# opencv/opencv_contrib

Hardware: AMD Instinct MI355X
Metric: frame-pairs/sec dense TV-L1 flow @1080p (higher is better)
Workload: dtype f32; 1 GPU; DualTVL1 dense flow, 1920x1080 CV_32FC1, 64 pairs/GPU/step (BASELINE configs[1]; 64 pairs/GPU = the per-GPU share of ~; warps=5, nscales=5, semantics=CPU_REF, math=fast, lanes=2

## Files before the change

### opencv_contrib_amd/csrc/mi_common.cpp

```cpp
#include "mi_common.h"
#include <vector>
#include <cstdlib>
#include <cstring>
#include <cstdio>
#include <mutex>

namespace mi {
static Tuning g_tuning;
static std::once_flag g_tuning_once;
static int env_int(const char *name, int dflt)
{
    const char *e = getenv(name);
    return e && *e ? atoi(e) : dflt;
}
#ifdef MIFLOW_EXPERIMENTS
#define EXP_INT(name, dflt) env_int(name, dflt)
#define EXP_ENV(name) getenv(name)
#else
#define EXP_INT(name, dflt) (dflt)
#define EXP_ENV(name) ((const char *)nullptr)
#endif
#ifndef MIFLOW_EXPERIMENTS
extern "C" char **environ;
static void warn_unread_switches()
{
    static const char *const known[] = {"MIFLOW_BF_W", "MIFLOW_CACHE_GB", "MIFLOW_CACHE_TOTAL_GB", "MIFLOW_FB_FUSE", "MIFLOW_FB_GROUP_MB", "MIFLOW_FB_NARROW",
                                        "MIFLOW_FB_PAIR", "MIFLOW_LANES", "MIFLOW_MULTI_RCCL", "MIFLOW_SURF_NMS0", "MIFLOW_SURF_POLY", "MIFLOW_SURF_STAGE_S",
                                        "MIFLOW_TB_HIST", "MIFLOW_TB_VERBOSE", "MIFLOW_TILE_MAXPX"};
    static const char *const foreign[] = {"MIFLOW_LIB", "MIFLOW_BENCH_", "MIFLOW_SWEEP_", "MIFLOW_BUILD_", "MIFLOW_EXTRA_", "MIFLOW_SLP_"};
    if (!environ) return;
    for (char **e = environ; *e; ++e) {
        if (strncmp(*e, "MIFLOW_", 7) != 0) continue;
        const char *eq = strchr(*e, '=');
        const size_t n = eq ? (size_t)(eq - *e) : strlen(*e);
        bool ok = false;
        for (const char *k : known) ok = ok || (strlen(k) == n && strncmp(k, *e, n) == 0);
        for (const char *k : foreign) ok = ok || strncmp(k, *e, strlen(k)) == 0;
        if (!ok) fprintf(stderr, "miflow: %.*s is not read by this library (tuning experiments exist in the -DMIFLOW_EXPERIMENTS build only); ignored\n", (int)n, *e);
    }
}
#endif
const Tuning &tuning()
{
    std::call_once(g_tuning_once, [] {
        Tuning &t = g_tuning;
#ifndef MIFLOW_EXPERIMENTS
        warn_unread_switches();
#endif
        t.x_skip = EXP_INT("MIFLOW_X_SKIP", 0);
        t.warp_tile = EXP_INT("MIFLOW_WARP_TILE", 32);
        if (t.warp_tile != 64 && t.warp_tile != 32 && t.warp_tile != 16) t.warp_tile = 32;
        t.warp_lds = EXP_INT("MIFLOW_WARP_LDS", 0);
        t.warp_fast = EXP_INT("MIFLOW_WARP_FAST", -1);
        t.warp_np = EXP_INT("MIFLOW_WARP_NP", 2);
        if (t.warp_np != 1 && t.warp_np != 4) t.warp_np = 2;
        t.tb_swz = EXP_INT("MIFLOW_TB_SWZ", 1);
        t.tb_p16 = EXP_INT("MIFLOW_TB_P16", 0);
        t.tb_nograd = EXP_INT("MIFLOW_TB_NOGRAD", 1);
        t.tb_skip_p = EXP_INT("MIFLOW_TB_SKIP_P", 1);
        t.tb_hist = env_int("MIFLOW_TB_HIST", 1);
        t.fb_poll = EXP_INT("MIFLOW_FB_POLL", 1);
        t.fb_ahead = EXP_INT("MIFLOW_FB_AHEAD", 1);
        t.tb_fw = EXP_INT("MIFLOW_TB_FW", 0);
        t.tb_jw = EXP_INT("MIFLOW_TB_JW", 2);
        if (t.tb_jw < 0 || t.tb_jw > 4) t.tb_jw = 2;
        t.tb_jw_spec = EXP_INT("MIFLOW_TB_JW_SPEC", 1);
        t.tb_ppl = t.tb_wps = t.tb_pf = -1;
        if (const char *v = EXP_ENV("MIFLOW_TB_VARIANT")) (void)sscanf(v, "%d,%d,%d", &t.tb_ppl, &t.tb_wps, &t.tb_pf);
        t.tb_force = EXP_ENV("MIFLOW_TB_FORCE") != nullptr;
        t.tb_plan_wps = EXP_INT("MIFLOW_TB_WPS", 0);
        t.tb_rows = EXP_INT("MIFLOW_TB_ROWS", 0);
        t.tb_verbose = getenv("MIFLOW_TB_VERBOSE") != nullptr;
        {
            const char *e = getenv("MIFLOW_TILE_MAXPX");
            t.tile_maxpx = e && *e ? atoll(e) : 2300000;
        }
        t.tile_variant = EXP_INT("MIFLOW_TILE_VARIANT", -1);
        t.tile_small_wgs = EXP_INT("MIFLOW_TILE_SMALL_WGS", 1024);
        t.tile_swz = EXP_INT("MIFLOW_TILE_SWZ", 1);
        t.warp_swz = EXP_INT("MIFLOW_WARP_SWZ", 1);
        t.tile_fb_block = EXP_INT("MIFLOW_TILE_FB_BLOCK", 10);
        t.tile_fb_model = EXP_INT("MIFLOW_TILE_FB_MODEL", 7);
        t.tile_spec = EXP_INT("MIFLOW_TILE_SPEC", 1);
        t.lanes = env_int("MIFLOW_LANES", 0);
        t.spec = EXP_INT("MIFLOW_SPEC", 1);
        t.exact_tb = EXP_INT("MIFLOW_EXACT_TB", 1);
        t.fb_tiled = EXP_INT("MIFLOW_FB_TILED", 1);
        t.sbm_wt = EXP_INT("MIFLOW_SBM_WT", 1);
        t.sbm_swz = EXP_INT("MIFLOW_SBM_SWZ", 1);
        t.sbm_texfuse = EXP_INT("MIFLOW_SBM_TEXFUSE", 1);
        t.fb_rows = EXP_INT("MIFLOW_FB_ROWS", 4) == 8 ? 8 : 4;
        t.fb_group_mb = env_int("MIFLOW_FB_GROUP_MB", 240);
        t.fb_fuse = env_int("MIFLOW_FB_FUSE", -1);
        t.fb_pair = env_int("MIFLOW_FB_PAIR", -1);
        t.fb_narrow = env_int("MIFLOW_FB_NARROW", -1);
        t.fb_swz = EXP_INT("MIFLOW_FB_SWZ", 1);
        t.fb_group_streams = EXP_INT("MIFLOW_FB_GROUP_STREAMS", 2);
        t.fb_poly_tiled = EXP_INT("MIFLOW_FB_POLY_TILED", 1);
        t.fb_direct = EXP_INT("MIFLOW_FB_DIRECT", 1);
        t.fb_blur_tiled = EXP_INT("MIFLOW_FB_BLUR_TILED", 1);
    });
    return g_tuning;
}

namespace {
struct BigBlock { void *p; size_t cap; int dev; hipEvent_t ready; };
std::mutex g_big_mu;
std::vector<BigBlock> g_big;
const size_t kBigMaxBlocks = 4;
size_t big_max_bytes()
{
    static const size_t v = [] {
        const char *e = getenv("MIFLOW_CACHE_GB");
        const long long gb = e && *e ? atoll(e) : 24;
        return (size_t)(gb < 0 ? 0 : gb) << 30;
    }();
    return v;
}
size_t big_max_bytes_total()
{
    static const size_t v = [] {
        const char *e = getenv("MIFLOW_CACHE_TOTAL_GB");
        if (e && *e) { const long long gb = atoll(e); return (size_t)(gb < 0 ? 0 : gb) << 30; }
        return 4 * big_max_bytes();
    }();
    return v;
}
}

int big_alloc(void **p, size_t bytes, size_t *capacity)
{
    int dev = 0;
    MI_HIP_TRY(hipGetDevice(&dev));
    {
        hipEvent_t ready = nullptr;
        bool hit = false;
        {
            std::lock_guard<std::mutex> lk(g_big_mu);
            int best = -1;
            for (size_t i = 0; i < g_big.size(); ++i)
                if (g_big[i].dev == dev && g_big[i].cap >= bytes && g_big[i].cap <= bytes + bytes / 2 + (64u << 20) &&
                    (best < 0 || g_big[i].cap < g_big[best].cap))
                    best = (int)i;
            if (best >= 0) {
                *p = g_big[best].p; *capacity = g_big[best].cap; ready = g_big[best].ready;
                g_big.erase(g_big.begin() + best);
                hit = true;
            }
        }
        if (hit) {
            if (ready) {
                const hipError_t we = hipEventSynchronize(ready);
                (void)hipEventDestroy(ready);
                if (we != hipSuccess) {
                    (void)hipGetLastError();
                    if (hipDeviceSynchronize() != hipSuccess) { (void)hipGetLastError(); (void)hipFree(*p); *p = nullptr; hit = false; }
                }
            }
            if (hit) return MI_OK;
        }
    }
    hipError_t e = hipMalloc(p, bytes);
    if (e != hipSuccess) {
        big_trim();
        e = hipMalloc(p, bytes);
    }
    if (e != hipSuccess) { set_error("hipMalloc of %zu bytes failed: %s", bytes, hipGetErrorString(e)); return MI_ERR_OOM; }
    *capacity = bytes;
    return MI_OK;
}

void big_free(void *p, size_t capacity, hipEvent_t ready, bool busy)
{
    if (!p) { if (ready) (void)hipEventDestroy(ready); return; }
    int dev = 0;
    void *drop = nullptr;
    if (hipGetDevice(&dev) == hipSuccess) {
        hipPointerAttribute_t at;
        const int cur = dev;
        if (hipPointerGetAttributes(&at, p) == hipSuccess) dev = at.device;
        if (dev != cur) (void)hipSetDevice(dev);
        bool idle = true;
        if (!ready && busy) idle = hipDeviceSynchronize() == hipSuccess;
        if (dev != cur) (void)hipSetDevice(cur);
        std::lock_guard<std::mutex> lk(g_big_mu);
        size_t total = capacity, all = capacity, blocks = 0;
        for (const BigBlock &b : g_big) {
            all += b.cap;
            if (b.dev == dev) { total += b.cap; ++blocks; }
        }
        if (idle && blocks < kBigMaxBlocks && total <= big_max_bytes() && all <= big_max_bytes_total()) {
            g_big.push_back({p, capacity, dev, ready});
            return;
        }
        if (ready) { (void)hipEventSynchronize(ready); (void)hipEventDestroy(ready); }
        drop = p;
    } else {
        if (ready) (void)hipEventDestroy(ready);
        drop = p;
    }
    const hipError_t fe = hipFree(drop);
    if (fe != hipSuccess) set_error("hipFree of a %zu-byte arena failed: %s", capacity, hipGetErrorString(fe));
}

void big_trim()
{
    std::vector<BigBlock> all;
    {
        std::lock_guard<std::mutex> lk(g_big_mu);
        all.swap(g_big);
    }
    int cur = 0;
    const bool have = hipGetDevice(&cur) == hipSuccess;
    for (const BigBlock &b : all) {
        if (b.ready) { (void)hipEventSynchronize(b.ready); (void)hipEventDestroy(b.ready); }
        (void)hipFree(b.p);
    }
    if (have) (void)hipSetDevice(cur);
}

int device_simds()
{
    static std::mutex mu;
    static int cache[64];
    int dev = 0;
    if (hipGetDevice(&dev) != hipSuccess || dev < 0 || dev >= 64) return 1024;
    std::lock_guard<std::mutex> lk(mu);
    if (!cache[dev]) {
        int cus = 0;
        if (hipDeviceGetAttribute(&cus, hipDeviceAttributeMultiprocessorCount, dev) != hipSuccess || cus <= 0) cus = 256;
        cache[dev] = 4 * cus;
    }
    return cache[dev];
}

static thread_local char g_err[512] = "";
void set_error(const char *fmt, ...)
{
    va_list ap;
    va_start(ap, fmt);
    vsnprintf(g_err, sizeof(g_err), fmt, ap);
    va_end(ap);
}
}

extern "C" {

const char *mi_last_error(void) { return mi::g_err; }
#ifdef MIFLOW_EXPERIMENTS
const char *mi_version(void) { return "miflow 0.1 (gfx950) +experiments"; }
#else
const char *mi_version(void) { return "miflow 0.1 (gfx950)"; }
#endif

int mi_device_count(void)
{
    int n = 0;
    if (hipGetDeviceCount(&n) != hipSuccess) return 0;
    return n;
}
int mi_set_device(int device) { MI_HIP_TRY(hipSetDevice(device)); return MI_OK; }
int mi_release_cached_memory(void) { mi::big_trim(); return MI_OK; }
int mi_get_device(int *device) { MI_REQUIRE(device, MI_ERR_BAD_ARG, "null device"); MI_HIP_TRY(hipGetDevice(device)); return MI_OK; }

int mi_malloc(void **dptr, size_t bytes)
{
    MI_REQUIRE(dptr, MI_ERR_BAD_ARG, "null dptr");
    MI_HIP_TRY(hipMalloc(dptr, bytes ? bytes : 1));
    return MI_OK;
}
int mi_malloc_pitch(void **dptr, size_t *step, size_t width_bytes, int rows)
{
    MI_REQUIRE(dptr && step && rows >= 0, MI_ERR_BAD_ARG, "bad mi_malloc_pitch arguments");
    const size_t st = rows > 1 ? (width_bytes + 255) / 256 * 256 : width_bytes;
    MI_HIP_TRY(hipMalloc(dptr, st * (size_t)(rows ? rows : 1) + 16));
    *step = st;
    return MI_OK;
}
int mi_free(void *dptr) { MI_HIP_TRY(hipFree(dptr)); return MI_OK; }
int mi_memcpy_h2d(void *dst, size_t dstep, const void *src, size_t sstep, size_t width_bytes, int rows, void *stream)
{
    MI_HIP_TRY(hipMemcpy2DAsync(dst, dstep, src, sstep, width_bytes, (size_t)rows, hipMemcpyHostToDevice, (hipStream_t)stream));
    return MI_OK;
}
int mi_memcpy_d2h(void *dst, size_t dstep, const void *src, size_t sstep, size_t width_bytes, int rows, void *stream)
{
    MI_HIP_TRY(hipMemcpy2DAsync(dst, dstep, src, sstep, width_bytes, (size_t)rows, hipMemcpyDeviceToHost, (hipStream_t)stream));
    return MI_OK;
}
int mi_memset(void *dst, size_t dstep, int value, size_t width_bytes, int rows, void *stream)
{
    MI_HIP_TRY(hipMemset2DAsync(dst, dstep, value, width_bytes, (size_t)rows, (hipStream_t)stream));
    return MI_OK;
}
int mi_stream_create(void **stream)
{
    MI_REQUIRE(stream, MI_ERR_BAD_ARG, "null stream");
    hipStream_t s;
    MI_HIP_TRY(hipStreamCreateWithFlags(&s, hipStreamNonBlocking));
    *stream = (void *)s;
    return MI_OK;
}
int mi_stream_destroy(void *stream) { MI_HIP_TRY(hipStreamDestroy((hipStream_t)stream)); return MI_OK; }
int mi_stream_synchronize(void *stream) { MI_HIP_TRY(hipStreamSynchronize((hipStream_t)stream)); return MI_OK; }

}
```

### opencv_contrib_amd/csrc/mi_common.h

```cpp
#pragma once
#include <vector>
#include <hip/hip_runtime.h>
#include <cstdarg>
#include <cstdio>
#include <cstring>
#include "miflow/c_api.h"

namespace mi {

void set_error(const char *fmt, ...);

#define MI_HIP_TRY(expr)                                                                  \
    do {                                                                                  \
        hipError_t _e = (expr);                                                           \
        if (_e != hipSuccess) {                                                           \
            mi::set_error("%s failed: %s (%s:%d)", #expr, hipGetErrorString(_e), __FILE__, __LINE__); \
            return _e == hipErrorOutOfMemory ? MI_ERR_OOM : MI_ERR_HIP;                   \
        }                                                                                 \
    } while (0)

#define MI_REQUIRE(cond, code, ...)        \
    do {                                   \
        if (!(cond)) {                     \
            mi::set_error(__VA_ARGS__);    \
            return (code);                 \
        }                                  \
    } while (0)

struct Tuning {
    int x_skip;
    int warp_tile;
    int warp_lds;
    int warp_fast;
    int warp_np;
    int tb_swz;
    int tb_p16;
    int tb_nograd;
    int tb_hist;
    int fb_poll;
    int fb_ahead;
    int tb_skip_p;
    int tb_fw;
    int tb_jw;
    int tb_jw_spec;
    int tb_ppl, tb_wps, tb_pf;
    int tb_force;
    int tb_plan_wps;
    int tb_rows;
    int tb_verbose;
    long long tile_maxpx;
    int tile_spec;
    int tile_variant;
    int tile_fb_block;
    int tile_fb_model;
    int tile_swz, warp_swz;
    int tile_small_wgs;
    int lanes;
    int exact_tb;
    int spec;
    int sbm_texfuse;
    int sbm_swz;
    int sbm_wt;
    int fb_rows, fb_swz;
    int fb_group_mb;
    int fb_fuse;
    int fb_pair;
    int fb_narrow;
    int fb_group_streams;
    int fb_poly_tiled;
    int fb_direct;
    int fb_blur_tiled;
    int fb_tiled;
};
const Tuning &tuning();
#ifdef MIFLOW_EXPERIMENTS
#define MI_EXP_ENV(name) getenv(name)
#else
#define MI_EXP_ENV(name) ((const char *)nullptr)
#endif

struct DevTmp {
    std::vector<void *> bufs;
    DevTmp() = default;
    DevTmp(const DevTmp &) = delete;
    DevTmp &operator=(const DevTmp &) = delete;
    ~DevTmp() { for (void *p : bufs) (void)hipFree(p); }
    template <class T>
    hipError_t alloc(T **out, size_t n)
    {
        void *p = nullptr;
        const hipError_t e = hipMalloc(&p, sizeof(T) * n);
        if (e == hipSuccess) bufs.push_back(p);
        *out = (T *)p;
        return e;
    }
};
int big_alloc(void **p, size_t bytes, size_t *capacity);
void big_free(void *p, size_t capacity, hipEvent_t ready = nullptr, bool busy = true);
void big_trim();
int device_simds();

static inline int div_up(int a, int b) { return (a + b - 1) / b; }
static inline int align_up(int a, int b) { return div_up(a, b) * b; }

struct PlaneF {
    float *p;
    int ld;
};

}
```

### opencv_contrib_amd/csrc/tvl1_api.cpp

```cpp
#include "tvl1_dev.h"
#include "mi_selftest.h"
#include <cfloat>
#include <algorithm>
#include <cmath>
#include <vector>
#include <chrono>
#include <sched.h>
#include <time.h>

using namespace mi;
using namespace mi::tvl1;

namespace {

constexpr double kFeedbackWaitLimitUs = 30e6;

struct LevelBuf {
    Geo g;
    float *I0 = nullptr, *I1 = nullptr;
    float *u[2][3] = {{nullptr, nullptr, nullptr}, {nullptr, nullptr, nullptr}};
};

struct SlotInfo { int scale, warp; };

template <class T, bool Host = false, unsigned HostFlags = 0>
struct GrowBuf {
    T *p = nullptr;
    size_t n = 0;
    GrowBuf() = default;
    GrowBuf(const GrowBuf &) = delete;
    ~GrowBuf() { release(); }
    int ensure(size_t want)
    {
        if (n >= want) return MI_OK;
        release();
        void *q = nullptr;
        if (Host) MI_HIP_TRY(hipHostMalloc(&q, sizeof(T) * want, HostFlags));
        else MI_HIP_TRY(hipMalloc(&q, sizeof(T) * want));
        p = (T *)q; n = want;
        return MI_OK;
    }
    void release()
    {
        if (p) (void)(Host ? hipHostFree(p) : hipFree(p));
        p = nullptr; n = 0;
    }
};

}

struct Lane {
    int capW = 0, capH = 0, capB = 0, capScales = 0;
    double capStep = 0;
    bool capGamma = false, capMedian = false;
    float *arena = nullptr;
    size_t arena_bytes = 0;
    std::vector<LevelBuf> L;
    float *scr[6] = {};
    float *pbuf[2][6] = {};
    GrowBuf<PtrTab> tab;
    std::vector<PtrTab> tab_host;
    GrowBuf<int2> S;
    GrowBuf<unsigned long long> E;
    GrowBuf<double> Pd;
    GrowBuf<int4> X;
    long long Q = 0;
    int ctlB = 0;
    GrowBuf<int> H;
    unsigned long long H_sig = 0;
    int H_par = 0;
    std::vector<SlotInfo> slots;
    GrowBuf<int2, true, hipHostMallocDefault> fb_host;
    hipEvent_t fb_ev = nullptr;
    GrowBuf<int, true, hipHostMallocCoherent | hipHostMallocMapped> fb_flag;
    int fb_seq = 0;
    std::vector<int> fb_hist;
    unsigned long long fb_hist_sig = 0;
    std::vector<hipEvent_t> ev_pool;
    struct Region { int e0, e1; long long launches; double bytes; int kind; int level; };
    std::vector<Region> regions;
    hipStream_t stream = nullptr;
    hipEvent_t done = nullptr;
    hipEvent_t idle_ev = nullptr;
    bool idle_valid = false;
    bool used = false;
};

struct mi_tvl1 {
    mi_tvl1_params P;
    int device = 0;
    float *cubic_tab = nullptr;
    static const int kMaxLanes = 4;
    Lane lane[kMaxLanes];
    hipEvent_t fork = nullptr;
    int last_nscales = 0, last_batch = 0, last_lanes = 1;
    int last_first[kMaxLanes + 1] = {};
    bool last_check = false;
    bool profiling = false;
};

void mi_tvl1_default_params(mi_tvl1_params *p)
{
    if (!p) return;
    p->tau = 0.25; p->lambda = 0.15; p->theta = 0.3; p->epsilon = 0.01; p->scale_step = 0.8; p->gamma = 0.0;
    p->nscales = 5; p->warps = 5; p->iterations = 300; p->use_initial_flow = 0;
    p->inner_iterations = 1; p->median_filtering = 1;
    p->semantics = MI_SEM_CPU_REF; p->exact_math = 0; p->time_block = 0; p->lanes = 0; p->stop_slack = 0; p->host_feedback = 0;
}

static const long long kMaxSlots = 4000000;

static int validate_params(const mi_tvl1_params *p)
{
    MI_REQUIRE(p, MI_ERR_BAD_ARG, "null params");
    MI_REQUIRE(p->nscales > 0 && p->nscales <= 32, MI_ERR_BAD_ARG, "nscales must be in [1,32] (CV_Assert nscales_ > 0)");
    MI_REQUIRE(p->warps >= 0 && p->warps <= 64, MI_ERR_BAD_ARG, "warps must be in [0,64]");
    MI_REQUIRE(p->iterations >= 0 && p->inner_iterations >= 0, MI_ERR_BAD_ARG, "negative iteration count");
    MI_REQUIRE((long long)p->iterations * p->inner_iterations <= kMaxSlots, MI_ERR_BAD_ARG,
               "iterations x inner_iterations must not exceed %lld", kMaxSlots);
    MI_REQUIRE(p->scale_step > 0 && p->scale_step < 1, MI_ERR_BAD_ARG, "scale_step must be in (0,1)");
    MI_REQUIRE(p->theta != 0, MI_ERR_BAD_ARG, "theta must be non-zero");
    MI_REQUIRE(p->semantics == MI_SEM_CPU_REF || p->semantics == MI_SEM_CUDA_COMPAT, MI_ERR_BAD_ARG, "bad semantics");
    MI_REQUIRE(p->median_filtering <= 1 || p->median_filtering == 3 || p->median_filtering == 5, MI_ERR_BAD_ARG,
               "medianFiltering must be 1 (off), 3 or 5 (cv::medianBlur on CV_32F)");
    MI_REQUIRE(p->lanes >= 0 && p->lanes <= 4, MI_ERR_BAD_ARG, "lanes must be 0 (automatic) or 1..4");
    MI_REQUIRE(p->stop_slack >= 0 && p->stop_slack <= 8, MI_ERR_BAD_ARG, "stop_slack must be in 0..8");
    MI_REQUIRE(p->host_feedback >= -1 && p->host_feedback <= 1, MI_ERR_BAD_ARG, "host_feedback must be -1, 0 or 1");
    return MI_OK;
}

int mi_tvl1_create(const mi_tvl1_params *p, mi_tvl1 **out)
{
    MI_REQUIRE(out, MI_ERR_BAD_ARG, "null out");
    *out = nullptr;
    mi_tvl1_params d;
    if (!p) { mi_tvl1_default_params(&d); p = &d; }
    int rc = validate_params(p);
    if (rc) return rc;
    int n = 0;
    if (hipGetDeviceCount(&n) != hipSuccess || n == 0) {
        set_error("no HIP device available: the miflow product path has no CPU fallback");
        return MI_ERR_NO_DEVICE;
    }
    mi_tvl1 *h = new mi_tvl1();
    h->P = *p;
    float tab[128];
    host_cubic_table(tab);
    auto upload = [&]() -> int {
        MI_HIP_TRY(hipGetDevice(&h->device));
        MI_HIP_TRY(hipMalloc((void **)&h->cubic_tab, sizeof(tab)));
        MI_HIP_TRY(hipMemcpy(h->cubic_tab, tab, sizeof(tab), hipMemcpyHostToDevice));
        return MI_OK;
    };
    if (const int rc = upload()) { mi_tvl1_destroy(h); return rc; }
    *out = h;
    return MI_OK;
}

int mi_tvl1_set_params(mi_tvl1 *h, const mi_tvl1_params *p)
{
    MI_REQUIRE(h, MI_ERR_BAD_ARG, "null handle");
    int rc = validate_params(p);
    if (rc) return rc;
    h->P = *p;
    return MI_OK;
}

int mi_tvl1_get_params(const mi_tvl1 *h, mi_tvl1_params *p)
{
    MI_REQUIRE(h && p, MI_ERR_BAD_ARG, "null argument");
    *p = h->P;
    return MI_OK;
}

static void free_arena(Lane &ln)
{
    if (ln.arena) {
        big_free(ln.arena, ln.arena_bytes, ln.idle_valid ? ln.idle_ev : nullptr, ln.used);
        if (ln.idle_valid) ln.idle_ev = nullptr;
    }
    ln.idle_valid = false;
    ln.used = false;
    ln.arena = nullptr;
    ln.L.clear();
}

int mi_tvl1_query_plan(int width, int height, int pairs_per_lane, int iterations_per_launch, int *kernel, int *rows_per_band)
{
    MI_REQUIRE(kernel && rows_per_band, MI_ERR_BAD_ARG, "null output");
    MI_REQUIRE(width > 0 && height > 0 && pairs_per_lane > 0 && iterations_per_launch > 0, MI_ERR_BAD_ARG, "bad plan query");
    int dev = 0;
    if (hipGetDevice(&dev) != hipSuccess) { set_error("no HIP device"); return MI_ERR_NO_DEVICE; }
    const Geo g{width, height, (width + 63) / 64 * 64, (long long)((width + 63) / 64 * 64) * height, pairs_per_lane};
    return tb_query_plan(iterations_per_launch, g, kernel, rows_per_band);
}

int mi_tvl1_set_profiling(mi_tvl1 *h, int enable)
{
    MI_REQUIRE(h, MI_ERR_BAD_ARG, "null handle");
    h->profiling = enable != 0;
    return MI_OK;
}

int mi_tvl1_get_profile(mi_tvl1 *h, double *ms_total, long long *launches, double *algo_bytes)
{
    return mi_tvl1_get_profile_kind(h, 0, ms_total, launches, algo_bytes);
}

int mi_tvl1_get_profile_kind(mi_tvl1 *h, int kind, double *ms_total, long long *launches, double *algo_bytes)
{
    return mi_tvl1_get_profile_level(h, kind, -1, ms_total, launches, algo_bytes);
}

int mi_tvl1_get_profile_level(mi_tvl1 *h, int kind, int level, double *ms_total, long long *launches, double *algo_bytes)
{
    MI_REQUIRE(h && ms_total && launches && algo_bytes, MI_ERR_BAD_ARG, "null argument");
    MI_REQUIRE(kind == 0 || kind == 1, MI_ERR_BAD_ARG, "kind must be 0 (iteration launches) or 1 (warp launches)");
    *ms_total = 0; *launches = 0; *algo_bytes = 0;
    for (int li = 0; li < h->last_lanes; ++li) {
        Lane &ln = h->lane[li];
        for (const auto &r : ln.regions) {
            if (r.kind != kind || (level >= 0 && r.level != level)) continue;
            MI_HIP_TRY(hipEventSynchronize(ln.ev_pool[r.e1]));
            float ms = 0.f;
            MI_HIP_TRY(hipEventElapsedTime(&ms, ln.ev_pool[r.e0], ln.ev_pool[r.e1]));
            *ms_total += ms; *launches += r.launches; *algo_bytes += r.bytes;
        }
    }
    return MI_OK;
}

void mi_tvl1_destroy(mi_tvl1 *h)
{
    if (!h) return;
    for (Lane &ln : h->lane) {
        for (hipEvent_t e : ln.ev_pool) (void)hipEventDestroy(e);
        free_arena(ln);
        if (ln.idle_ev) { (void)hipEventDestroy(ln.idle_ev); ln.idle_ev = nullptr; }
        if (ln.done) (void)hipEventDestroy(ln.done);
        if (ln.fb_ev) (void)hipEventDestroy(ln.fb_ev);
        if (ln.stream) (void)hipStreamDestroy(ln.stream);
    }
    if (h->fork) (void)hipEventDestroy(h->fork);
    if (h->cubic_tab) (void)hipFree(h->cubic_tab);
    delete h;
}

static int ensure_arena(const mi_tvl1_params &P, Lane &ln, const TvPlan &pl, int W, int H, int B)
{
    const bool gam = P.gamma != 0.0, med = pl.median != 0;
    if (!(ln.arena && ln.capW == W && ln.capH == H && ln.capB >= B && ln.capScales == P.nscales && ln.capStep == P.scale_step &&
          ln.capGamma == gam && ln.capMedian == med)) {
        free_arena(ln);
        void *blk = nullptr;
        if (const int rc = big_alloc(&blk, pl.arena.total * sizeof(float), &ln.arena_bytes)) return rc;
        ln.arena = (float *)blk;
        const auto at = [&](size_t o) { return o == kNoPlane ? nullptr : ln.arena + o; };
        ln.L.resize(pl.geo.size());
        for (size_t l = 0; l < pl.geo.size(); ++l) {
            ln.L[l].I0 = at(pl.arena.lv[l][0]); ln.L[l].I1 = at(pl.arena.lv[l][1]);
            for (int k = 0; k < 6; ++k) ln.L[l].u[k / 3][k % 3] = at(pl.arena.lv[l][2 + k]);
        }
        for (int k = 0; k < 6; ++k) ln.scr[k] = at(pl.arena.scr[k]);
        for (int k = 0; k < 12; ++k) ln.pbuf[k / 6][k % 6] = at(pl.arena.p[k]);
        ln.capGamma = gam; ln.capMedian = med; ln.capW = W; ln.capH = H; ln.capB = B; ln.capScales = P.nscales; ln.capStep = P.scale_step;
    }
    for (size_t l = 0; l < pl.geo.size(); ++l) ln.L[l].g = pl.geo[l];
    return MI_OK;
}

static int check_pair(const mi_mat *I0, const mi_mat *I1, const mi_mat *flow, const mi_mat *I0ref)
{
    MI_REQUIRE(I0 && I1 && flow, MI_ERR_BAD_ARG, "null matrix");
    MI_REQUIRE(I0->data && I1->data && flow->data, MI_ERR_BAD_ARG, "null data pointer");
    MI_REQUIRE(I0->type == MI_8UC1 || I0->type == MI_32FC1, MI_ERR_BAD_TYPE, "I0 must be CV_8UC1 or CV_32FC1");
    MI_REQUIRE(I0->rows == I1->rows && I0->cols == I1->cols, MI_ERR_BAD_SIZE, "I0.size() != I1.size()");
    MI_REQUIRE(I0->type == I1->type, MI_ERR_BAD_TYPE, "I0.type() != I1.type()");
    MI_REQUIRE(flow->type == MI_32FC2, MI_ERR_BAD_TYPE, "flow must be CV_32FC2");
    MI_REQUIRE(flow->rows == I0->rows && flow->cols == I0->cols, MI_ERR_BAD_SIZE, "flow.size() != I0.size()");
    MI_REQUIRE(I0->rows >= 3 && I0->cols >= 3, MI_ERR_BAD_SIZE, "image must be at least 3x3");
    MI_REQUIRE((long long)((I0->cols + 63) / 64 * 64) * I0->rows * 4 < (1LL << 32), MI_ERR_BAD_SIZE,
               "image too large: a float plane of it must stay below 4 GiB");
    const size_t es = I0->type == MI_8UC1 ? 1 : 4;
    MI_REQUIRE(I0->step >= (size_t)I0->cols * es && I1->step >= (size_t)I1->cols * es, MI_ERR_BAD_ARG, "step < cols*elemSize");
    MI_REQUIRE(flow->step >= (size_t)flow->cols * 8, MI_ERR_BAD_ARG, "flow step < cols*8");
    if (es == 4) MI_REQUIRE(I0->step % 4 == 0 && I1->step % 4 == 0 && ((uintptr_t)I0->data % 4) == 0 && ((uintptr_t)I1->data % 4) == 0,
                            MI_ERR_BAD_ARG, "float images must be 4-byte aligned");
    MI_REQUIRE(flow->step % 8 == 0 && ((uintptr_t)flow->data % 8) == 0, MI_ERR_BAD_ARG, "flow must be 8-byte aligned");
    MI_REQUIRE(I0->rows == I0ref->rows && I0->cols == I0ref->cols && I0->type == I0ref->type, MI_ERR_BAD_SIZE,
               "all pairs of a batch must share size and type");
    return MI_OK;
}

const TvKnobs &mi::tvl1::tv_knobs()
{
    static const TvKnobs k = [] {
        const Tuning &t = tuning();
        TvKnobs v{};
        v.tile_maxpx = t.tile_maxpx; v.tile_spec = t.tile_spec; v.tile_variant = t.tile_variant; v.tile_small_wgs = t.tile_small_wgs;
        v.tile_variants = std::min(tile_variants(), (int)(sizeof(v.tile_rows) / sizeof(v.tile_rows[0])));
        for (int i = 0; i < v.tile_variants; ++i) v.tile_rows[i] = tile_shape_rows(i);
        v.tile_fb_block = t.tile_fb_block; v.tile_fb_model = t.tile_fb_model;
        v.tb_force = t.tb_force != 0; v.tb_nograd = t.tb_nograd; v.tb_jw = t.tb_jw; v.tb_ppl = t.tb_ppl; v.tb_jw_spec = t.tb_jw_spec;
        v.tb_fw = t.tb_fw; v.tb_skip_p = t.tb_skip_p; v.tb_hist = t.tb_hist; v.spec = t.spec; v.exact_tb = t.exact_tb;
        v.fb_poll = t.fb_poll; v.fb_ahead = t.fb_ahead; v.warp_fast = t.warp_fast; v.warp_lds = t.warp_lds; v.x_skip = t.x_skip;
        return v;
    }();
    return k;
}

static int ensure_buffers(const TvPlan &pl, Lane &ln, int B, const mi_mat *I0s, const mi_mat *I1s, mi_mat *flows, hipStream_t st)
{
    int rc;
    if ((rc = ln.tab.ensure(B))) return rc;
    ln.tab_host.resize(B);
    for (int i = 0; i < B; ++i)
        ln.tab_host[i] = PtrTab{I0s[i].data, I1s[i].data, flows[i].data, (long long)I0s[i].step, (long long)I1s[i].step, (long long)flows[i].step};
    MI_HIP_TRY(hipMemcpyAsync(ln.tab.p, ln.tab_host.data(), sizeof(PtrTab) * B, hipMemcpyHostToDevice, st));
    if (pl.check) {
        MI_REQUIRE(pl.Q <= kMaxSlots, MI_ERR_BAD_ARG, "scales x warps x iterations = %lld control slots exceed the limit of %lld", pl.Q, kMaxSlots);
        if (ln.Q < pl.Q || ln.ctlB < B) {
            const size_t n = (size_t)pl.Q * B;
            if ((rc = ln.S.ensure(n)) || (rc = ln.E.ensure(n)) || (rc = ln.Pd.ensure(n)) || (rc = ln.X.ensure(n))) return rc;
            ln.Q = pl.Q; ln.ctlB = B;
        }
        MI_HIP_TRY(hipMemsetAsync(ln.E.p, 0, sizeof(unsigned long long) * (size_t)ln.Q * B, st));
        MI_HIP_TRY(hipMemsetAsync(ln.S.p, 0, sizeof(int2) * (size_t)ln.Q * B, st));
    }
    if (pl.hist) {
        const int nw = (int)pl.warp[0].size();
        const size_t h_n = (size_t)pl.used * nw * B;
        if (ln.H.n < 2 * h_n) ln.H_sig = 0;
        if ((rc = ln.H.ensure(2 * h_n))) return rc;
        if (ln.H_sig != pl.hist_sig) {
            MI_HIP_TRY(hipMemsetAsync(ln.H.p, 0, sizeof(int) * ln.H.n, st));
            ln.H_sig = pl.hist_sig;
        }
        if (ln.fb_hist_sig != pl.hist_sig || ln.fb_hist.size() != (size_t)pl.used * nw) {
            ln.fb_hist.assign((size_t)pl.used * nw, 0);
            ln.fb_hist_sig = pl.hist_sig;
        }
        ln.H_par ^= 1;
    }
    if (pl.fb) {
        const bool fresh = ln.fb_flag.n < 2 * (size_t)B;
        if ((rc = ln.fb_host.ensure(2 * (size_t)B)) || (rc = ln.fb_flag.ensure(2 * (size_t)B))) return rc;
        if (fresh) memset(ln.fb_flag.p, 0, sizeof(int) * ln.fb_flag.n);
        if (!ln.fb_ev) MI_HIP_TRY(hipEventCreateWithFlags(&ln.fb_ev, hipEventDisableTiming));
    }
    return MI_OK;
}

namespace {

struct Run {
    mi_tvl1 *h;
    Lane &ln;
    const TvPlan &pl;
    const TvKnobs &K;
    hipStream_t st;
    int B;
    size_t ev_used = 0;
    Ctl ctl;
    IterPlanes planes;
    float *grad = nullptr;
    float l_t, theta, taut;
    int q = 0, q_last = -1, e_next = 0;
    int q_settle_prev = -1, q_settle_scale = -1;
    int fb_prev_warp = 2, fb_prev_scale = 2;
    int cur = 0;
    bool first_of_scale = true;
    bool pre_warped = false;
};

int record(Run &r, int *idx)
{
    if (r.ev_used == r.ln.ev_pool.size()) {
        hipEvent_t e;
        MI_HIP_TRY(hipEventCreate(&e));
        r.ln.ev_pool.push_back(e);
    }
    *idx = (int)r.ev_used++;
    MI_HIP_TRY(hipEventRecord(r.ln.ev_pool[*idx], r.st));
    return MI_OK;
}

int enqueue_pyramid(Run &r, int type)
{
    const mi_tvl1_params &P = r.h->P;
    Lane &ln = r.ln;
    const int ns = r.pl.used, B = r.B;
    int rc = convert(ln.tab.p, type, ln.L[0].I0, ln.L[0].I1, ln.L[0].g, r.st);
    if (rc) return rc;
    if (P.use_initial_flow && (rc = unpack_flow(ln.tab.p, ln.L[0].u[0][0], ln.L[0].u[0][1], ln.L[0].g, r.st))) return rc;
    const float one3[3] = {1.f, 1.f, 1.f};
    for (size_t s = 1; s < ln.L.size(); ++s) {
        const LevelBuf &c = ln.L[s - 1];
        const float *src[3][2] = {{c.I0, nullptr}, {c.I1, nullptr}, {nullptr, nullptr}};
        float *dst[3] = {ln.L[s].I0, ln.L[s].I1, nullptr};
        rc = resize(P.semantics, 2, src, 1, dst, c.g, ln.L[s].g, P.scale_step, P.scale_step, one3, nullptr, 0, r.st);
        if (rc) return rc;
        if ((int)s >= ns) break;
        if (P.use_initial_flow) {
            const float *us[3][2] = {{c.u[0][0], nullptr}, {c.u[0][1], nullptr}, {nullptr, nullptr}};
            float *ud[3] = {ln.L[s].u[0][0], ln.L[s].u[0][1], nullptr};
            const float post[3] = {(float)P.scale_step, (float)P.scale_step, 1.f};
            rc = resize(P.semantics, 2, us, 1, ud, c.g, ln.L[s].g, P.scale_step, P.scale_step, post, nullptr, 0, r.st);
            if (rc) return rc;
        }
    }
    const LevelBuf &Lc = ln.L[ns - 1];
    const size_t bytes = sizeof(float) * (size_t)Lc.g.ps * B;
    if (!P.use_initial_flow) {
        MI_HIP_TRY(hipMemsetAsync(Lc.u[0][0], 0, bytes, r.st));
        MI_HIP_TRY(hipMemsetAsync(Lc.u[0][1], 0, bytes, r.st));
    }
    if (P.gamma != 0.0) MI_HIP_TRY(hipMemsetAsync(Lc.u[0][2], 0, bytes, r.st));
    return MI_OK;
}

int launch_warp(Run &r, const LevelBuf &Lv, bool ahead)
{
    const float *u1v[2] = {Lv.u[0][0], Lv.u[1][0]}, *u2v[2] = {Lv.u[0][1], Lv.u[1][1]};
    Ctl c = r.ctl;
    c.q_prev = r.q_last;
    c.need_done = ahead ? 1 : 0;
    const bool dev_cur = ahead || (r.pl.check && !r.first_of_scale);
    return warp_fused(r.h->P.semantics, r.pl.fast_warp, -1, Lv.I0, Lv.I1, u1v, u2v, nullptr, r.ln.scr[2], r.ln.scr[3],
                      r.grad, r.ln.scr[5], r.h->cubic_tab, Lv.g, dev_cur ? &c : nullptr, r.cur, r.st);
}

int run_blocked(Run &r, LevelBuf &Lv, const TvWarp &w, long long *nlaunch)
{
    const int sem = r.h->P.semantics;
    float *const mu1[2] = {Lv.u[0][0], Lv.u[1][0]}, *const mu2[2] = {Lv.u[0][1], Lv.u[1][1]};
    const int nb = (int)w.blocks.size();
    int rc;
    for (int no = 0; no < w.outer; ++no) {
        if (r.pl.median && (rc = median_flow(r.pl.median, mu1, mu2, r.ln.scr[0], r.ln.scr[1], Lv.g, nullptr, r.cur, r.st))) return rc;
        for (int k = 0; k < nb; ++k) {
            ++*nlaunch;
            if (w.skip_iterations) { r.first_of_scale = false; continue; }
            const bool last_pass = w.skip_p_last && no == w.outer - 1 && k == nb - 1;
            rc = w.form == TvForm::ExactBlocked ? iterate_tb_exact(w.blocks[k], r.planes, Lv.g, r.l_t, r.theta, r.taut, r.first_of_scale, r.cur, r.st)
               : w.fused ? iterate_tb_fused(sem, Lv.I0, Lv.I1, r.h->cubic_tab, w.blocks[k], r.planes, Lv.g, r.l_t, r.theta, r.taut,
                                            r.first_of_scale, r.cur, r.st, last_pass)
                         : iterate_tb(w.blocks[k], r.planes, Lv.g, r.l_t, r.theta, r.taut, r.first_of_scale, r.cur, 0, r.st, last_pass);
            if (rc) return rc;
            r.cur ^= 1;
            r.first_of_scale = false;
        }
    }
    return MI_OK;
}

int run_per_iteration(Run &r, LevelBuf &Lv, int s, int wp, long long *nlaunch)
{
    const mi_tvl1_params &P = r.h->P;
    const int mf = r.pl.median;
    float *const mu1[2] = {Lv.u[0][0], Lv.u[1][0]}, *const mu2[2] = {Lv.u[0][1], Lv.u[1][1]};
    int rc;
    for (int it = 0; it < r.pl.iters; ++it) {
        ++*nlaunch;
        if (mf && it % P.inner_iterations == 0) {
            Ctl mc = r.ctl;
            mc.q_prev = r.q_last; mc.first_of_warp = (it == 0); mc.reset_cur = r.first_of_scale;
            if ((rc = median_flow(mf, mu1, mu2, r.ln.scr[0], r.ln.scr[1], Lv.g, r.pl.check ? &mc : nullptr, r.cur, r.st))) return rc;
        }
        if (r.pl.check) {
            Ctl ic = r.ctl;
            ic.q = r.q; ic.q_prev = r.q_last; ic.first_of_warp = (it == 0); ic.reset_cur = r.first_of_scale; ic.n = it;
            rc = iterate(P.exact_math != 0, r.planes, Lv.g, r.l_t, r.theta, r.taut, r.first_of_scale, &ic, 0, r.st);
            r.ln.slots.push_back({s, wp});
            r.q_last = r.q++;
        } else {
            rc = iterate(P.exact_math != 0, r.planes, Lv.g, r.l_t, r.theta, r.taut, r.first_of_scale, nullptr, r.cur, r.st);
            r.cur ^= 1;
        }
        if (rc) return rc;
        r.first_of_scale = false;
    }
    return MI_OK;
}

struct Feedback { bool all = true, all_before = true; int n_most = 0; };

int poll_feedback(Run &r, int seq, Feedback *f)
{
    const int *flag = r.ln.fb_flag.p;
    for (int b = 0; b < r.B; ++b) {
        int v = 0;
        const auto t_wait0 = std::chrono::steady_clock::now();
        for (long long spin = 0;; ++spin) {
            v = __atomic_load_n(flag + 2 * b, __ATOMIC_ACQUIRE);
            if ((v >> 2) == seq) break;
            if ((spin & 63) != 63) {
#if defined(__x86_64__) || defined(__i386__)
                __builtin_ia32_pause();
#endif
                continue;
            }
            const double waited_us = std::chrono::duration<double, std::micro>(std::chrono::steady_clock::now() - t_wait0).count();
            if (waited_us < 20.0) continue;
            const hipError_t qe = hipStreamQuery(r.st);
            if (qe != hipErrorNotReady) {
                v = __atomic_load_n(flag + 2 * b, __ATOMIC_ACQUIRE);
                if ((v >> 2) == seq) break;
                MI_HIP_TRY(qe);
                MI_REQUIRE(false, MI_ERR_HIP, "host feedback: launch finished without publishing its decision");
            }
            MI_REQUIRE(waited_us < kFeedbackWaitLimitUs, MI_ERR_HIP, "host feedback: no decision from the device within %.0f s", kFeedbackWaitLimitUs * 1e-6);
            if (waited_us < 2000.0) sched_yield();
            else { struct timespec ts_ = {0, 50000}; nanosleep(&ts_, nullptr); }
        }
        f->all_before = f->all_before && (v & 2);
        f->all = f->all && (v & 1);
        f->n_most = std::max(f->n_most, flag[2 * b + 1]);
    }
    return MI_OK;
}

int copy_feedback(Run &r, Feedback *f)
{
    Lane &ln = r.ln;
    MI_HIP_TRY(hipMemcpy2DAsync(ln.fb_host.p, 2 * sizeof(int2), ln.S.p + (r.q_last - 1), sizeof(int2) * (size_t)ln.Q, 2 * sizeof(int2),
                                (size_t)r.B, hipMemcpyDeviceToHost, r.st));
    MI_HIP_TRY(hipEventRecord(ln.fb_ev, r.st));
    MI_HIP_TRY(hipEventSynchronize(ln.fb_ev));
    for (int b = 0; b < r.B; ++b) {
        f->all_before = f->all_before && (ln.fb_host.p[2 * b].y & MI_SLOT_DONE);
        f->all = f->all && (ln.fb_host.p[2 * b + 1].y & MI_SLOT_DONE);
    }
    return MI_OK;
}

int run_spec(Run &r, LevelBuf &Lv, const TvWarp &w, int s, int wp, long long *nlaunch)
{
    const TvPlan &pl = r.pl;
    Lane &ln = r.ln;
    const int nw = (int)pl.warp[s].size();
    int rc, hprev = 0;
    if (pl.fb_poll && pl.hist) {
        int &hc = ln.fb_hist[(size_t)s * nw + wp];
        hprev = hc;
        hc = 0;
    }
    const std::vector<int> plan = spec_blocks(w, Lv.g, hprev, r.K);
    int t_after = 0;
    for (int v : plan) t_after += v;
    SpecK sk;
    memset(&sk, 0, sizeof(sk));
    sk.X = ln.X.p; sk.iters = pl.iters;
    sk.q_hist = wp > 0 ? r.q_settle_prev : r.q_settle_scale;
    spec_hist_fraction(wp, &sk.hist_num, &sk.hist_den);
    sk.slack = r.h->P.stop_slack;
    if (pl.hist) {
        const size_t o = ((size_t)s * nw + wp) * r.B, half = ln.H.n / 2;
        sk.h_in = ln.H.p + (size_t)(ln.H_par ^ 1) * half + o;
        sk.h_out = ln.H.p + (size_t)ln.H_par * half + o;
    }
    if (r.first_of_scale) {
        const size_t n = (size_t)Lv.g.ps * r.B;
        if ((rc = zero_planes4(ln.pbuf[0], n, r.st))) return rc;
        float *const p3[4] = {ln.pbuf[0][4], ln.pbuf[0][5], ln.pbuf[0][4], ln.pbuf[0][5]};
        if (r.h->P.gamma != 0.0 && (rc = zero_planes4(p3, n, r.st))) return rc;
    }
    int e_prev = 0;
    int fb_next = pl.fb ? spec_first_poll(plan, hprev, wp > 0 ? r.fb_prev_warp : r.fb_prev_scale) : -1;
    int fb_done_at = (int)plan.size();
    for (size_t k = 0; k <= plan.size(); ++k) {
        const bool last = k == plan.size();
        const int T = last ? plan.back() : plan[k];
        if (!last) t_after -= T;
        Ctl a = r.ctl;
        a.q = r.q; a.q_prev = r.q_last; a.first_of_warp = (k == 0); a.reset_cur = (k == 0 && r.first_of_scale); a.n = 0;
        sk.e0_prev = e_prev; sk.final_launch = last ? 1 : 0; sk.t_after = t_after;
        if (pl.fb_poll) {
            ln.fb_seq = (ln.fb_seq + 1) & 0x0fffffff;
            sk.fb_flag = ln.fb_flag.p; sk.fb_seq = ln.fb_seq;
        }
        MI_REQUIRE((long long)r.e_next + T <= ln.Q && r.q < ln.Q, MI_ERR_BAD_ARG,
                   "speculative steps: error-sum slot %d + %d or launch slot %d beyond the %lld slots sized for this calc", r.e_next, T, r.q, ln.Q);
        if ((rc = iterate_tb_spec(T, r.planes, Lv.g, r.l_t, r.theta, r.taut, false, a, sk, r.e_next, r.st))) return rc;
        ln.slots.push_back({s, wp});
        r.q_last = r.q++;
        ++*nlaunch;
        e_prev = r.e_next;
        if (!last) r.e_next += T;
        if (!pl.fb || last || (int)k != fb_next) continue;
        const bool ahead = pl.fb_poll && r.K.fb_ahead != 0 && r.K.x_skip == 0 && !r.h->profiling && wp + 1 < nw;
        if (ahead && (rc = launch_warp(r, Lv, true))) return rc;
        Feedback f;
        if ((rc = pl.fb_poll ? poll_feedback(r, ln.fb_seq, &f) : copy_feedback(r, &f))) return rc;
        if (f.all) {
            r.pre_warped = ahead;
            if (pl.fb_poll && pl.hist) ln.fb_hist[(size_t)s * nw + wp] = f.n_most;
            fb_done_at = f.all_before ? (int)k - 1 : (int)k;
            break;
        }
        fb_next = (int)k + 2;
    }
    if (pl.fb) {
        r.fb_prev_warp = fb_done_at;
        if (wp == 0) r.fb_prev_scale = fb_done_at;
    }
    r.q_settle_prev = r.q_last;
    if (wp == 0) r.q_settle_scale = r.q_last;
    r.first_of_scale = false;
    return MI_OK;
}

int run_warp(Run &r, LevelBuf &Lv, int s, int wp)
{
    const TvWarp &w = r.pl.warp[s][wp];
    const Geo &g = Lv.g;
    const bool prof = r.h->profiling;
    int rc, w0 = -1, w1 = -1, e0 = -1, e1 = -1;
    r.planes.g = r.grad = w.nograd ? nullptr : r.ln.scr[4];
    if (prof && (rc = record(r, &w0))) return rc;
    if (r.pre_warped) r.pre_warped = false;
    else if (w.warp_launch && (rc = launch_warp(r, Lv, false))) return rc;
    if (prof && !w.fused) {
        if ((rc = record(r, &w1))) return rc;
        r.ln.regions.push_back({w0, w1, 1, 44.0 * g.w * g.h * r.B, 1, s});
    }
    if (prof && r.pl.iters > 0 && (rc = record(r, &e0))) return rc;
    long long nlaunch = 0;
    switch (w.form) {
    case TvForm::Blocked:
    case TvForm::ExactBlocked: rc = run_blocked(r, Lv, w, &nlaunch); break;
    case TvForm::Spec: rc = run_spec(r, Lv, w, s, wp, &nlaunch); break;
    case TvForm::PerIter: rc = run_per_iteration(r, Lv, s, wp, &nlaunch); break;
    }
    if (rc) return rc;
    if (e0 >= 0) {
        if ((rc = record(r, &e1))) return rc;
        r.ln.regions.push_back({e0, e1, nlaunch, 64.0 * g.w * g.h * r.B * r.pl.iters, 0, s});
    }
    return MI_OK;
}

int zoom_or_pack(Run &r, int s)
{
    const mi_tvl1_params &P = r.h->P;
    const LevelBuf &Lv = r.ln.L[s];
    Ctl ec = r.ctl;
    ec.q_prev = r.q_last;
    const Ctl *dev = r.pl.check && !r.first_of_scale ? &ec : nullptr;
    if (s == 0) {
        const float *u1v[2] = {Lv.u[0][0], Lv.u[1][0]}, *u2v[2] = {Lv.u[0][1], Lv.u[1][1]};
        return pack_flow(r.ln.tab.p, u1v, u2v, Lv.g, dev, r.cur, r.st);
    }
    const LevelBuf &Lf = r.ln.L[s - 1];
    const bool gam = P.gamma != 0.0;
    const float *us[3][2] = {{Lv.u[0][0], Lv.u[1][0]}, {Lv.u[0][1], Lv.u[1][1]}, {gam ? Lv.u[0][2] : nullptr, gam ? Lv.u[1][2] : nullptr}};
    float *ud[3] = {Lf.u[0][0], Lf.u[0][1], gam ? Lf.u[0][2] : nullptr};
    const float post[3] = {(float)(1.0 / P.scale_step), (float)(1.0 / P.scale_step), 1.f};
    return resize(P.semantics, gam ? 3 : 2, us, 2, ud, Lv.g, Lf.g, (double)Lf.g.w / Lv.g.w, (double)Lf.g.h / Lv.g.h, post, dev, r.cur, r.st);
}

}

static int lane_calc(mi_tvl1 *h, Lane &ln, int n, const mi_mat *I0s, const mi_mat *I1s, mi_mat *flows, hipStream_t st, int *ns_out)
{
    struct Mark {
        Lane &l; hipStream_t s;
        ~Mark()
        {
            if (!l.arena) return;
            l.used = true; l.idle_valid = false;
            hipStreamCaptureStatus cs = hipStreamCaptureStatusNone;
            if (hipStreamIsCapturing(s, &cs) != hipSuccess || cs != hipStreamCaptureStatusNone) { (void)hipGetLastError(); return; }
            if (!l.idle_ev && hipEventCreateWithFlags(&l.idle_ev, hipEventDisableTiming) != hipSuccess) { l.idle_ev = nullptr; (void)hipGetLastError(); return; }
            if (hipEventRecord(l.idle_ev, s) == hipSuccess) l.idle_valid = true; else (void)hipGetLastError();
        }
    } mark{ln, st};
    const mi_tvl1_params &P = h->P;
    hipStreamCaptureStatus cap_st = hipStreamCaptureStatusNone;
    const bool capturing = hipStreamIsCapturing(st, &cap_st) == hipSuccess && cap_st != hipStreamCaptureStatusNone;
    const TvPlan pl = tv_make_plan(TvShape{I0s[0].cols, I0s[0].rows, n, I0s[0].type, P, h->last_lanes, capturing}, tv_knobs());
    int rc = ensure_arena(P, ln, pl, I0s[0].cols, I0s[0].rows, n);
    if (rc || (rc = ensure_buffers(pl, ln, n, I0s, I1s, flows, st))) return rc;
    *ns_out = pl.used;
    ln.slots.clear();
    ln.regions.clear();

    Run r{h, ln, pl, tv_knobs(), st, n};
    memset(&r.ctl, 0, sizeof(r.ctl));
    r.ctl.S = ln.S.p; r.ctl.E = ln.E.p; r.ctl.Q = (int)ln.Q; r.ctl.P = ln.Pd.p;
    r.ctl.sched = P.semantics == MI_SEM_CUDA_COMPAT ? 1 : 0;
    r.l_t = (float)(P.lambda * P.theta); r.taut = (float)(P.tau / P.theta); r.theta = (float)P.theta;
    if ((rc = enqueue_pyramid(r, I0s[0].type))) return rc;
    for (int s = pl.used - 1; s >= 0; --s) {
        LevelBuf &Lv = ln.L[s];
        IterPlanes &ip = r.planes;
        ip.ix = ln.scr[2]; ip.iy = ln.scr[3]; ip.rc = ln.scr[5]; ip.gamma = (float)P.gamma;
        for (int k = 0; k < 2; ++k) { for (int j = 0; j < 3; ++j) ip.u[k][j] = Lv.u[k][j]; for (int j = 0; j < 6; ++j) ip.p[k][j] = ln.pbuf[k][j]; }
        ip.err_u3 = P.semantics == MI_SEM_CPU_REF ? 1 : 0;
        r.cur = 0; r.first_of_scale = true; r.pre_warped = false;
        const double se = P.epsilon * P.epsilon * (double)(Lv.g.w * Lv.g.h);
        r.ctl.thr = P.semantics == MI_SEM_CPU_REF ? (double)(float)se : se;
        for (int wp = 0; wp < P.warps; ++wp)
            if ((rc = run_warp(r, Lv, s, wp))) return rc;
        if ((rc = zoom_or_pack(r, s))) return rc;
    }
    return MI_OK;
}

int mi_tvl1_calc_batch(mi_tvl1 *h, int n, const mi_mat *I0s, const mi_mat *I1s, mi_mat *flows, void *stream_)
{
    MI_REQUIRE(h, MI_ERR_BAD_ARG, "null handle");
    MI_REQUIRE(n > 0 && I0s && I1s && flows, MI_ERR_BAD_ARG, "empty batch");
    hipStream_t st = (hipStream_t)stream_;
    for (int i = 0; i < n; ++i) {
        int rc = check_pair(&I0s[i], &I1s[i], &flows[i], &I0s[0]);
        if (rc) return rc;
    }
    int lanes = h->P.lanes > 0 ? h->P.lanes : (tuning().lanes > 0 ? tuning().lanes : (n >= 4 ? 2 : 1));
    if (lanes > mi_tvl1::kMaxLanes) lanes = mi_tvl1::kMaxLanes;
    if (lanes > n) lanes = n;
    int ns = 0;
    h->last_check = h->P.epsilon > 0.0 && h->P.iterations * h->P.inner_iterations > 0;
    h->last_batch = n; h->last_lanes = lanes;
    for (int i = 0; i <= lanes; ++i) h->last_first[i] = (int)((long long)n * i / lanes);
    if (lanes == 1) {
        int rc = lane_calc(h, h->lane[0], n, I0s, I1s, flows, st, &ns);
        if (rc) return rc;
    } else {
        if (!h->fork) MI_HIP_TRY(hipEventCreateWithFlags(&h->fork, hipEventDisableTiming));
        for (int li = 1; li < lanes; ++li) {
            Lane &ln = h->lane[li];
            if (!ln.stream) MI_HIP_TRY(hipStreamCreateWithFlags(&ln.stream, hipStreamNonBlocking));
            if (!ln.done) MI_HIP_TRY(hipEventCreateWithFlags(&ln.done, hipEventDisableTiming));
        }
        MI_HIP_TRY(hipEventRecord(h->fork, st));
        int rc_first = MI_OK;
        auto note = [&](hipError_t e) {
            if (e != hipSuccess && !rc_first) { set_error("HIP error in the lane fork / join: %s", hipGetErrorString(e)); rc_first = MI_ERR_HIP; }
            return e == hipSuccess;
        };
        for (int li = lanes - 1; li >= 0; --li) {
            Lane &ln = h->lane[li];
            const int off = h->last_first[li], cnt = h->last_first[li + 1] - off;
            hipStream_t ls = li > 0 ? ln.stream : st;
            const bool forked = li == 0 || note(hipStreamWaitEvent(ln.stream, h->fork, 0));
            if (forked && !rc_first) {
                const int rc = lane_calc(h, ln, cnt, I0s + off, I1s + off, flows + off, ls, &ns);
                if (rc && !rc_first) rc_first = rc;
            }
        }
        for (int li = 1; li < lanes; ++li) {
            Lane &ln = h->lane[li];
            if (!(note(hipEventRecord(ln.done, ln.stream)) && note(hipStreamWaitEvent(st, ln.done, 0)))) (void)hipStreamSynchronize(ln.stream);
        }
        if (rc_first) return rc_first;
    }
    h->last_nscales = ns;
    if (ns < h->P.nscales) h->P.nscales = ns;
    return MI_OK;
}

int mi_tvl1_calc(mi_tvl1 *h, const mi_mat *I0, const mi_mat *I1, mi_mat *flow, void *stream)
{
    return mi_tvl1_calc_batch(h, 1, I0, I1, flow, stream);
}

static int read_slots(mi_tvl1 *h, int pair, hipStream_t stream, const Lane **lane, std::vector<int2> *S, std::vector<int4> *X,
                      int cap_launches = -1)
{
    int li = 0;
    while (li + 1 < h->last_lanes && pair >= h->last_first[li + 1]) ++li;
    const Lane &ln = h->lane[li];
    const size_t off = (size_t)(pair - h->last_first[li]) * ln.Q;
    const int nq = (int)ln.slots.size();
    MI_REQUIRE(cap_launches < 0 || nq <= cap_launches, MI_ERR_BAD_ARG, "capacity too small");
    *lane = &ln;
    S->resize(nq);
    MI_HIP_TRY(hipStreamSynchronize(stream));
    MI_HIP_TRY(hipMemcpy(S->data(), ln.S.p + off, sizeof(int2) * nq, hipMemcpyDeviceToHost));
    if (X) {
        X->resize(nq);
        if (ln.X.p) MI_HIP_TRY(hipMemcpy(X->data(), ln.X.p + off, sizeof(int4) * nq, hipMemcpyDeviceToHost));
    }
    return MI_OK;
}

int mi_tvl1_last_iterations(mi_tvl1 *h, int pair, int *nscales_used, int *iters, int cap, void *stream)
{
    MI_REQUIRE(h && iters && nscales_used, MI_ERR_BAD_ARG, "null argument");
    MI_REQUIRE(pair >= 0 && pair < h->last_batch, MI_ERR_BAD_ARG, "pair index out of range");
    const int ns = h->last_nscales, nw = h->P.warps;
    MI_REQUIRE(cap >= ns * nw, MI_ERR_BAD_ARG, "iters capacity too small");
    *nscales_used = ns;
    for (int i = 0; i < ns * nw; ++i) iters[i] = 0;
    if (!h->last_check) {
        for (int i = 0; i < ns * nw; ++i) iters[i] = h->P.iterations * h->P.inner_iterations;
        return MI_OK;
    }
    const Lane *ln = nullptr;
    std::vector<int2> S;
    if (const int rc = read_slots(h, pair, (hipStream_t)stream, &ln, &S, nullptr)) return rc;
    for (size_t i = 0; i < S.size(); ++i) {
        const int k = (S[i].y >> 8) & 0xff;
        iters[ln->slots[i].scale * nw + ln->slots[i].warp] += k ? k : (S[i].y & 1);
    }
    return MI_OK;
}

int miflow_selftest_tvl1_slots(mi_tvl1 *h, int pair, int *out_host, int cap_launches, void *stream)
{
    MI_REQUIRE(h && out_host, MI_ERR_BAD_ARG, "null argument");
    MI_REQUIRE(pair >= 0 && pair < h->last_batch, MI_ERR_BAD_ARG, "pair out of range");
    if (!h->last_check) return 0;
    const Lane *ln = nullptr;
    std::vector<int2> S;
    std::vector<int4> X;
    if (const int rc = read_slots(h, pair, (hipStream_t)stream, &ln, &S, &X, cap_launches)) return rc;
    const int nq = (int)S.size();
    for (int i = 0; i < nq; ++i) {
        int *o = out_host + 8 * i;
        o[0] = ln->slots[i].scale; o[1] = ln->slots[i].warp; o[2] = S[i].x; o[3] = S[i].y;
        o[4] = X[i].x; o[5] = X[i].y; o[6] = X[i].z; o[7] = X[i].w;
    }
    return nq;
}
```

### opencv_contrib_amd/csrc/tvl1_dev.h

```cpp
#pragma once
#include "mi_common.h"
#include "tvl1_plan.h"

namespace mi {
namespace tvl1 {

const TvKnobs &tv_knobs();

struct Ctl {
    int2 *S;
    unsigned long long *E;
    int Q;
    int q;
    int q_prev;
    int first_of_warp;
    int reset_cur;
    double thr;
    double *P;
    int sched;
    int n;
    int need_done;
};

#define MI_SLOT_FLIP 1
#define MI_SLOT_CHECKED 2
#define MI_SLOT_DONE 4
#define MI_SLOT_ITERS(y) (((y) >> 8) & 0xff)

struct PtrTab {
    const void *a, *b;
    void *out;
    long long step_a, step_b, step_out;
};

struct IterPlanes {
    const float *ix, *iy, *g, *rc;
    float *u[2][3];
    float *p[2][6];
    float gamma;
    int err_u3;
};

int convert(const PtrTab *tab_dev, int type, float *I0, float *I1, const Geo &g, hipStream_t s);
int zero_planes4(float *const p[4], size_t n, hipStream_t s);
int unpack_flow(const PtrTab *tab_dev, float *u1, float *u2, const Geo &g, hipStream_t s);
int pack_flow(const PtrTab *tab_dev, const float *u1[2], const float *u2[2], const Geo &g,
              const Ctl *ctl, int cur_host, hipStream_t s);
int resize(int semantics, int nplanes, const float *const src[3][2], int src_sets, float *const dst[3],
           const Geo &gs, const Geo &gd, double inv_scale_x, double inv_scale_y,
           const float post_scale[3], const Ctl *ctl, int cur_host, hipStream_t s);
int gradient(const float *src, float *dx, float *dy, const Geo &g, hipStream_t s);
int median_flow(int ksize, float *const u1[2], float *const u2[2], float *tmp1, float *tmp2, const Geo &g, const Ctl *ctl, int cur_host,
                hipStream_t s);
int pack3(const float *a, const float *b, const float *c, float *pk, const Geo &g, hipStream_t s);
int warp(int semantics, const float *I0, const float *pk, const float *u1[2], const float *u2[2], float *I1w,
         float *I1wx, float *I1wy, float *grad, float *rho, const float *cubic_tab_dev, const Geo &g, const Ctl *ctl,
         int cur_host, hipStream_t s);
int warp_fused(int semantics, bool fast, int lds, const float *I0, const float *I1, const float *u1[2], const float *u2[2], float *I1w, float *I1wx,
               float *I1wy, float *grad, float *rho, const float *cubic_tab_dev, const Geo &g, const Ctl *ctl, int cur_host,
               hipStream_t s);
int iterate(bool exact, const IterPlanes &pl, const Geo &g, float l_t, float theta, float taut,
            bool p_zero, const Ctl *ctl, int cur_host, hipStream_t s);

int iterate_tb(int T, const IterPlanes &pl, const Geo &g, float l_t, float theta, float taut, bool p_zero,
               int cur, int rows_per_band, hipStream_t s, bool skip_p_out = false, bool independent_waves = false);
int iterate_tb_fused(int semantics, const float *I0, const float *I1, const float *cubic_tab_dev, int T, const IterPlanes &pl, const Geo &g,
                     float l_t, float theta, float taut, bool p_zero, int cur, hipStream_t s, bool skip_p_out);
int iterate_tile(int variant, int nit, const IterPlanes &pl, const Geo &g, float l_t, float theta, float taut, bool p_zero, int cur,
                 hipStream_t s);
int tile_owned_rows();
int tile_shape_rows(int variant);
int tb_query_plan(int T, const Geo &g, int *kernel, int *rows);
int tile_variants();
int iterate_tb_exact(int T, const IterPlanes &pl, const Geo &g, float l_t, float theta, float taut, bool p_zero, int cur, hipStream_t s,
                     int rows_per_band = 0);
bool tb_kernel_exists(int kind, int T, bool gam, bool nograd);
struct SpecK {
    int4 *X;
    int e0_prev;
    int final_launch;
    int iters;
    int t_after;
    int q_hist;
    int hist_num, hist_den;
    int slack;
    const int *h_in;
    int *h_out;
    int *fb_flag;
    int fb_seq;
};

int iterate_tile_spec(int T, const IterPlanes &pl, const Geo &g, float l_t, float theta, float taut, const Ctl &ctl, const SpecK &sk, int e0,
                      hipStream_t s, int variant = -1);
int iterate_tb_spec(int T, const IterPlanes &pl, const Geo &g, float l_t, float theta, float taut, bool p_zero, const Ctl &ctl,
                    const SpecK &sk, int e0, hipStream_t s, int rows_per_band = 0);
int dbg_lane_shift(int *out_dev, hipStream_t s);
int tb_jw_fault(int *fault_host);

void host_cubic_table(float tab[128]);

}
}
```

### opencv_contrib_amd/csrc/tvl1_plan.h

```cpp
#pragma once
#include "miflow/c_api.h"
#include <algorithm>
#include <array>
#include <cmath>
#include <cstddef>
#include <initializer_list>
#include <vector>

namespace mi {
namespace tvl1 {

struct Geo {
    int w, h, ld;
    long long ps;
    int batch;
};

constexpr int kTbMaxBlock = 10;
constexpr int kTbExactMaxBlock = 5;
constexpr int kTileMaxBlock = 10;
constexpr double kLargeLevel = 12e6;

struct TvKnobs {
    long long tile_maxpx;
    int tile_spec;
    int tile_variant, tile_small_wgs, tile_variants, tile_rows[8];
    int tile_fb_block, tile_fb_model;
    bool tb_force;
    int tb_nograd, tb_jw, tb_ppl, tb_jw_spec;
    int tb_fw;
    int tb_skip_p, tb_hist, spec, exact_tb;
    int fb_poll, fb_ahead;
    int warp_fast, warp_lds, x_skip;
};


inline bool tile_eligible(const Geo &g, const TvKnobs &K)
{
    return K.tile_maxpx > 0 && (long long)g.w * g.h * g.batch <= K.tile_maxpx;
}
inline bool runs_on_tiles(const Geo &g, int T, const TvKnobs &K, bool spec = false)
{
    return tile_eligible(g, K) && T <= kTileMaxBlock && (spec ? K.tile_spec != 0 : !K.tb_force);
}
inline bool tb_nograd_ok(int T, const Geo &g, const TvKnobs &K)
{
    return K.tb_nograd && T == 10 && K.tb_jw == 2 && K.tb_ppl < 0 && !runs_on_tiles(g, T, K);
}
inline bool tb_spec_nograd_ok(const Geo &g, const TvKnobs &K)
{
    return K.tb_nograd && K.tb_jw >= 2 && K.tb_jw_spec && !(tile_eligible(g, K) && K.tile_spec != 0);
}
inline bool tb_fused_ok(int T, const Geo &g, int semantics, bool fast_warp, const TvKnobs &K)
{
    if (!K.tb_fw || !tb_nograd_ok(T, g, K) || g.w < 6 || g.h < 6) return false;
    return (semantics == MI_SEM_CPU_REF && !fast_warp) || (semantics == MI_SEM_CUDA_COMPAT && fast_warp);
}

inline int tile_auto_variant(const Geo &g, bool spec, const TvKnobs &K)
{
    if (K.tile_variant >= 0) return K.tile_variant < K.tile_variants ? K.tile_variant : 0;
    constexpr int M = kTileMaxBlock, LW = 64, STRIDE = LW - 2 * M;
    const long long nstrips = g.w <= LW - M ? 1 : 1 + (g.w - (LW - M) + STRIDE - 1) / STRIDE;
    const long long wgs = nstrips * ((g.h + (64 - 2 * M) - 1) / (64 - 2 * M)) * g.batch;
    return wgs < (long long)K.tile_small_wgs * (spec ? 2 : 1) ? 1 : 0;
}
inline int tile_rows_for(const Geo &g, const TvKnobs &K) { return K.tile_rows[tile_auto_variant(g, true, K)]; }

inline std::vector<int> greedy_blocks(int n, int cap, std::initializer_list<int> sup)
{
    std::vector<int> blocks;
    for (int left = n; left > 0; left -= blocks.back()) {
        int t = 1;
        for (int c : sup) if (c <= left && c <= cap) t = std::max(t, c);
        blocks.push_back(t);
    }
    return blocks;
}
inline std::vector<int> tb_plan(int n, int cap, const TvKnobs &K)
{
    static const int sup[] = {1, 2, 3, 4, 5, 6, 8, 10};
    static const double cost[11] = {0, 15.6, 9.4, 6.6, 4.65, 3.9, 3.7, 0, 2.83, 0, 2.54};
    std::vector<int> blocks;
    if (n <= 0) return blocks;
    if (K.tb_force) return greedy_blocks(n, cap, {1, 2, 3, 4, 5, 6, 8, 10});
    std::vector<double> best(n + 1, 1e300);
    std::vector<int> pick(n + 1, 1);
    best[0] = 0;
    for (int i = 1; i <= n; ++i)
        for (int t : sup) {
            if (t > i || t > cap) continue;
            const double c = best[i - t] + t * cost[t];
            if (c < best[i]) { best[i] = c; pick[i] = t; }
        }
    for (int i = n; i > 0; i -= pick[i]) blocks.push_back(pick[i]);
    return blocks;
}
inline std::vector<int> tb_plan_level(const Geo &g, int n, int cap, bool gam, const TvKnobs &K)
{
    if (!tile_eligible(g, K) || K.tb_force) return gam ? greedy_blocks(n, cap, {10, 5, 2, 1}) : tb_plan(n, cap, K);
    return greedy_blocks(n, std::min(cap, kTileMaxBlock), {1, 2, 3, 4, 5, 6, 7, 8, 9, 10});
}
inline std::vector<int> tb_spec_plan(int n, int list, int B, const TvKnobs &K)
{
    std::vector<int> blocks;
    const int want = n + (n > 10 ? 30 : n > 1 ? 10 : 0);
    const int tile = (B <= 2 && K.tile_fb_block > 0) ? std::min(K.tile_fb_block, kTileMaxBlock) : kTileMaxBlock;
    for (int sum = 0; sum < want; sum += blocks.back())
        blocks.push_back(list == 3 ? tile : n <= 5 ? 5 : list == 0 ? 10 : blocks.size() < 12 ? 5 : 10);
    return blocks;
}


struct TvShape {
    int W, H, B, type;
    mi_tvl1_params P;
    int lanes;
    bool capturing;
};

enum class TvForm {
    Blocked,
    ExactBlocked,
    Spec,
    PerIter,
};

struct TvWarp {
    TvForm form;
    std::vector<int> blocks;
    int outer;
    bool on_tiles;
    bool nograd;
    bool fused;
    bool warp_launch;
    bool skip_iterations;
    bool skip_p_last;
};

constexpr size_t kNoPlane = (size_t)-1;
struct TvArena {
    size_t total = 0;
    std::vector<std::array<size_t, 8>> lv;
    size_t scr[6];
    size_t p[12];
};

struct TvPlan {
    std::vector<Geo> geo;
    int used;
    TvArena arena;
    int iters;
    int median;
    bool check, spec, hist;
    bool fb, fb_poll;
    bool fast_warp;
    long long Q;
    unsigned long long hist_sig;
    std::vector<std::vector<TvWarp>> warp;
};

inline std::vector<Geo> tv_levels(const mi_tvl1_params &P, int W, int H, int B, int *used)
{
    std::vector<Geo> geo;
    int w = W, h = H;
    *used = 0;
    for (int s = 0; s < P.nscales; ++s) {
        if (s > 0) {
            w = (int)std::lrint(w * P.scale_step);
            h = (int)std::lrint(h * P.scale_step);
            if (w < 1 || h < 1) break;
        }
        geo.push_back(Geo{w, h, (w + 63) / 64 * 64, (long long)((w + 63) / 64 * 64) * h, B});
        if (s > 0 && (w < 16 || h < 16)) break;
        *used = s + 1;
    }
    return geo;
}

inline TvArena tv_arena(const std::vector<Geo> &geo, int B, bool gam, bool med)
{
    TvArena a;
    auto take = [&](size_t nfloats) { const size_t o = a.total; a.total += (nfloats + 63) / 64 * 64; return o; };
    for (const Geo &g : geo) {
        const size_t n = (size_t)g.ps * B;
        std::array<size_t, 8> o;
        o[0] = take(n); o[1] = take(n);
        for (int k = 0; k < 6; ++k) o[2 + k] = (k % 3 == 2 && !gam) ? kNoPlane : take(n);
        a.lv.push_back(o);
    }
    const size_t nfull = (size_t)geo[0].ps * B;
    for (int k = 0; k < 6; ++k) a.scr[k] = (k < 2 && !med) ? kNoPlane : take(nfull);
    for (int k = 0; k < 12; ++k) a.p[k] = (k % 6 >= 4 && !gam) ? kNoPlane : take(nfull);
    return a;
}

inline int spec_tile_block(int hprev, const Geo &g, const TvKnobs &K)
{
    const double px = (double)g.w * g.h * g.batch, TR = (double)tile_rows_for(g, K);
    int best = 10;
    double best_cost = 1e30;
    for (int bl : {4, 7, 10}) {
        const double passes = (double)((hprev + bl - 1) / bl);
        const double lanes = px * 64.0 / (64.0 - 2.0 * bl) * TR / (TR - 2.0 * bl);
        const double cost = passes * (double)K.tile_fb_model + lanes * (passes * 10.8e-6 + (double)hprev * 2.4e-6);
        if (cost < best_cost) { best_cost = cost; best = bl; }
    }
    return best;
}
inline std::vector<int> spec_blocks(const TvWarp &w, const Geo &g, int hprev, const TvKnobs &K, int bl = 0)
{
    std::vector<int> plan = w.blocks;
    if (!w.on_tiles || hprev < 1 || plan.empty()) return plan;
    if (K.tile_fb_model != 0) {
        if (bl <= 0) bl = spec_tile_block(hprev, g, K);
        int total = 0;
        for (int v : plan) total += v;
        plan.assign((size_t)((total + bl - 1) / bl), bl);
    } else if (hprev <= 7) plan[0] = hprev <= 4 ? 4 : 7;
    return plan;
}
inline int spec_first_poll(const std::vector<int> &plan, int hprev, int prev_done)
{
    if (hprev <= 0) return std::max(1, prev_done);
    int kq = 0, sum = 0;
    while (kq < (int)plan.size() && (sum += plan[kq]) < hprev) ++kq;
    return std::max(1, std::min(kq + 1, (int)plan.size() - 1));
}
inline void spec_hist_fraction(int wp, int *num, int *den)
{
    *num = wp == 0 ? 7 : wp == 1 ? 9 : 4;
    *den = wp == 0 ? 10 : wp == 1 ? 20 : 5;
}

inline TvPlan tv_make_plan(const TvShape &S, const TvKnobs &K)
{
    const mi_tvl1_params &P = S.P;
    const int B = S.B;
    const bool gam = P.gamma != 0.0;
    TvPlan p;
    p.geo = tv_levels(P, S.W, S.H, B, &p.used);
    p.median = P.median_filtering > 1 ? P.median_filtering : 0;
    p.arena = tv_arena(p.geo, B, gam, p.median != 0);
    p.iters = P.iterations * P.inner_iterations;
    p.check = P.epsilon > 0.0 && p.iters > 0;
    p.spec = p.check && !P.exact_math && P.time_block != 1 && !p.median && K.spec != 0;
    p.hist = p.spec && K.tb_hist != 0;
    p.fb = p.spec && S.lanes == 1 && P.host_feedback >= 0 && (P.host_feedback == 1 || B <= 2) && !S.capturing;
    p.fb_poll = p.fb && K.fb_poll != 0;
    p.fast_warp = !P.exact_math && (K.warp_fast > 0 || (K.warp_fast < 0 && P.semantics == MI_SEM_CUDA_COMPAT));
    p.hist_sig = 1469598103934665603ull;
    for (long long v : {(long long)S.W, (long long)S.H, (long long)B, (long long)p.used, (long long)P.warps, (long long)p.iters, (long long)S.type})
        p.hist_sig = (p.hist_sig ^ (unsigned long long)v) * 1099511628211ull;

    const long long sw = (long long)p.used * P.warps;
    p.Q = sw * p.iters;
    std::vector<int> spec_list[4];
    if (p.spec) {
        long long e_max = 0, l_max = 0;
        for (int k = 0; k < 4; ++k) {
            spec_list[k] = tb_spec_plan(p.iters, k, B, K);
            long long t = 0;
            for (int v : spec_list[k]) t += v;
            e_max = std::max(e_max, t);
            l_max = std::max(l_max, (long long)spec_list[k].size() + 1);
        }
        e_max += 2 * (long long)std::max(kTileMaxBlock, kTbMaxBlock);
        p.Q = std::max(sw * e_max, sw * l_max);
    }

    const bool blocked = !p.check && !P.exact_math && P.time_block != 1;
    const bool exact_blocked = !p.check && P.exact_math && P.time_block != 1 && !gam && !p.median && K.exact_tb != 0;
    p.warp.resize(p.used);
    for (int s = 0; s < p.used; ++s) {
        const Geo &g = p.geo[s];
        TvWarp w{};
        w.outer = 1;
        if (blocked) {
            w.form = TvForm::Blocked;
            w.outer = p.median ? P.iterations : 1;
            w.blocks = tb_plan_level(g, p.median ? P.inner_iterations : p.iters, P.time_block > 0 ? P.time_block : kTbMaxBlock, gam, K);
            w.nograd = !w.blocks.empty();
            for (int v : w.blocks) w.nograd = w.nograd && (gam || tb_nograd_ok(v, g, K));
            w.fused = !gam && w.nograd && w.blocks.size() == 1 && !p.median && K.x_skip == 0 && K.warp_lds == 0 &&
                      tb_fused_ok(w.blocks[0], g, P.semantics, p.fast_warp, K);
            w.skip_iterations = K.x_skip == 2;
        } else if (exact_blocked) {
            w.form = TvForm::ExactBlocked;
            const int cap = P.time_block > 0 ? std::min(P.time_block, kTbExactMaxBlock) : kTbExactMaxBlock;
            for (int left = p.iters; left > 0; left -= w.blocks.back()) w.blocks.push_back(std::min(left, cap));
        } else if (p.spec) {
            w.form = TvForm::Spec;
            w.on_tiles = tile_eligible(g, K) && K.tile_spec != 0;
            w.nograd = gam || tb_spec_nograd_ok(g, K);
        } else
            w.form = TvForm::PerIter;
        p.warp[s].assign(P.warps, w);
        for (int wp = 0; wp < P.warps; ++wp) {
            TvWarp &x = p.warp[s][wp];
            if (x.form == TvForm::Spec)
                x.blocks = spec_list[x.on_tiles ? 3 : wp > 0 ? 2 : ((double)g.w * g.h * B >= kLargeLevel ? 0 : 1)];
            x.warp_launch = !x.fused && !(K.x_skip == 1 && wp > 0);
            x.skip_p_last = x.form == TvForm::Blocked && K.tb_skip_p && wp == P.warps - 1 && !p.median;
        }
    }
    return p;
}

}
}
```

### opencv_contrib_amd/csrc/tvl1_tb_dev.h

```cpp
#pragma once
#include "tvl1_dev.h"
#include "tvl1_warp_dev.h"

namespace mi {
namespace tvl1 {

__device__ __forceinline__ float dpp_from_prev(float v)
{
    return __int_as_float(__builtin_amdgcn_update_dpp(0, __float_as_int(v), 0x138, 0xf, 0xf, true));
}
__device__ __forceinline__ float dpp_from_next(float v)
{
    return __int_as_float(__builtin_amdgcn_update_dpp(0, __float_as_int(v), 0x130, 0xf, 0xf, true));
}

__device__ __forceinline__ float dpp_from_prev_fill(float v, float fill)
{
    return __int_as_float(__builtin_amdgcn_update_dpp(__float_as_int(fill), __float_as_int(v), 0x138, 0xf, 0xf, false));
}
__device__ __forceinline__ float dpp_from_next_fill(float v, float fill)
{
    return __int_as_float(__builtin_amdgcn_update_dpp(__float_as_int(fill), __float_as_int(v), 0x130, 0xf, 0xf, false));
}

template <int PPL>
struct Dyn {
    float u1[PPL], u2[PPL], p11[PPL], p12[PPL], p21[PPL], p22[PPL];
};
template <int PPL>
struct Dyn3 {
    float u3[PPL], p31[PPL], p32[PPL];
};
template <int PPL>
struct Stat {
    float ix[PPL], iy[PPL], rg[PPL], rc[PPL];
};

struct TbArgs {
    IterPlanes pl;
    Geo g;
    float l_t, theta, taut;
    int rows_per_band;
    int cur;
    int swz, nstrips;
    int skip_p_out;
    CtlK ctl;
    int e0;
    SpecK sk;
    const float *fI0, *fI1, *ftab;
};

#define ERR_FIX_SCALE 16777216.0

__device__ __forceinline__ bool spec_settle(const CtlK &ck, const SpecK &sk, int T, int b, bool writer, int &cur, int &nit_out, bool &record)
{
    int base = 0, done = 0, n = 0, replay = 0, accepted = 0, pbase = 0, done_before = 0;
    double prev = 0.0;
    float e_last = 0.f, e_before = 0.f;
    if (ck.q_prev >= 0) {
        const long long sp = (long long)b * ck.Q + ck.q_prev;
        const int2 sl = ck.S[sp];
        pbase = sl.x ^ (sl.y & MI_SLOT_FLIP);
        base = pbase;
        if (!ck.first_of_warp) {
            const int4 px = sk.X[sp];
            prev = ck.P[sp];
            n = px.x;
            e_last = __int_as_float(px.z);
            if (sl.y & MI_SLOT_DONE) {
                done = 1; done_before = 1;
            } else if (px.y > 0) {
                const int pn = px.y;
                int kk = 0, conv = 0;
                for (int t = 0; t < pn; ++t) {
                    const int na = n + t;
                    const bool calc = !ck.sched || ((na & 1) && prev < ck.thr);
                    const double e = (double)ck.E[(long long)b * ck.Q + sk.e0_prev + t] * (1.0 / ERR_FIX_SCALE);
                    e_before = e_last;
                    e_last = (float)(e / ck.thr);
                    if (calc) {
                        prev = e;
                        if (!(e > ck.thr)) { kk = t + 1; conv = 1; break; }
                    } else {
                        prev -= ck.thr;
                    }
                }
                if (conv && kk + sk.slack < pn) {
                    replay = kk; accepted = kk; n += kk; done = 1;
                } else {
                    base = pbase ^ 1; accepted = pn; n += pn;
                    done = conv || n >= sk.iters;
                }
            }
        }
    }
    if (ck.reset_cur) base = pbase = 0;
    int nit = 0;
    if (replay) {
        nit = replay;
    } else if (!done && !sk.final_launch) {
        int pred = T;
        const int hist = sk.h_in ? sk.h_in[b] : 0;
        if (!ck.sched && hist > n) {
            pred = hist - n;
        } else if (!ck.sched) {
            if (ck.first_of_warp) {
                if (sk.q_hist >= 0) pred = (sk.X[(long long)b * ck.Q + sk.q_hist].x * sk.hist_num) / sk.hist_den;
            } else if (e_before > e_last && e_last > 1.f) {
                pred = (int)ceilf(__logf(e_last) / __logf(e_before / e_last));
            } else if (e_last > 0.f) {
                pred = 2;
            }
        }
        const int hi = min(T, sk.iters - n), lo = max(1, sk.iters - n - sk.t_after);
        nit = max(lo, min(hi, pred));
        record = true;
    }
    if (writer) {
        const long long sq = (long long)b * ck.Q + ck.q;
        ck.S[sq] = make_int2(replay ? pbase : base, (replay ? MI_SLOT_FLIP : 0) | (done ? MI_SLOT_DONE : 0) | (accepted << 8));
        ck.P[sq] = prev;
        sk.X[sq] = make_int4(n, record ? nit : 0, __float_as_int(e_last), 0);
        if (sk.h_out) sk.h_out[b] = n;
        if (sk.fb_flag) {
            sk.fb_flag[2 * b + 1] = n;
            __hip_atomic_store(sk.fb_flag + 2 * b, (sk.fb_seq << 2) | (done_before << 1) | done, __ATOMIC_RELEASE, __HIP_MEMORY_SCOPE_SYSTEM);
        }
    }
    if (nit == 0) return false;
    cur = replay ? pbase : base;
    nit_out = nit;
    return true;
}

template <int PPL>
__device__ __forceinline__ void lds_put(float *slot, int lane, const Stat<PPL> &s)
{
    float *q = slot + lane * PPL;
    if (PPL == 1) {
        q[0] = s.ix[0]; q[64] = s.iy[0]; q[128] = s.rg[0]; q[192] = s.rc[0];
    } else if (PPL == 2) {
        *reinterpret_cast<float2 *>(q) = make_float2(s.ix[0], s.ix[1]);
        *reinterpret_cast<float2 *>(q + 128) = make_float2(s.iy[0], s.iy[1]);
        *reinterpret_cast<float2 *>(q + 256) = make_float2(s.rg[0], s.rg[1]);
        *reinterpret_cast<float2 *>(q + 384) = make_float2(s.rc[0], s.rc[1]);
    } else {
        *reinterpret_cast<float4 *>(q) = make_float4(s.ix[0], s.ix[1], s.ix[2], s.ix[3]);
        *reinterpret_cast<float4 *>(q + 256) = make_float4(s.iy[0], s.iy[1], s.iy[2], s.iy[3]);
        *reinterpret_cast<float4 *>(q + 512) = make_float4(s.rg[0], s.rg[1], s.rg[2], s.rg[3]);
        *reinterpret_cast<float4 *>(q + 768) = make_float4(s.rc[0], s.rc[1], s.rc[2], s.rc[3]);
    }
}
template <int PPL>
__device__ __forceinline__ void lds_get(const float *slot, int lane, Stat<PPL> &s)
{
    const float *q = slot + lane * PPL;
    if (PPL == 1) {
        s.ix[0] = q[0]; s.iy[0] = q[64]; s.rg[0] = q[128]; s.rc[0] = q[192];
    } else if (PPL == 2) {
        float2 a = *reinterpret_cast<const float2 *>(q), b = *reinterpret_cast<const float2 *>(q + 128);
        float2 c = *reinterpret_cast<const float2 *>(q + 256), d = *reinterpret_cast<const float2 *>(q + 384);
        s.ix[0] = a.x; s.ix[1] = a.y; s.iy[0] = b.x; s.iy[1] = b.y;
        s.rg[0] = c.x; s.rg[1] = c.y; s.rc[0] = d.x; s.rc[1] = d.y;
    } else {
        float4 a = *reinterpret_cast<const float4 *>(q), b = *reinterpret_cast<const float4 *>(q + 256);
        float4 c = *reinterpret_cast<const float4 *>(q + 512), d = *reinterpret_cast<const float4 *>(q + 768);
        s.ix[0] = a.x; s.ix[1] = a.y; s.ix[2] = a.z; s.ix[3] = a.w;
        s.iy[0] = b.x; s.iy[1] = b.y; s.iy[2] = b.z; s.iy[3] = b.w;
        s.rg[0] = c.x; s.rg[1] = c.y; s.rg[2] = c.z; s.rg[3] = c.w;
        s.rc[0] = d.x; s.rc[1] = d.y; s.rc[2] = d.z; s.rc[3] = d.w;
    }
}

template <int PPL>
__device__ __forceinline__ void finish_static(Stat<PPL> &st)
{
#pragma unroll
    for (int j = 0; j < PPL; ++j) st.rg[j] = __builtin_amdgcn_rcpf(fmaxf(st.rg[j], 1e-30f));
}

}
}
```

### opencv_contrib_amd/csrc/tvl1_tbr_kernels.hip

```cpp
#include "tvl1_tb_dev.h"
#include "tvl1_warp_px.h"
#include <utility>
#include <cstdlib>
#include <cstdio>
#include <vector>

namespace mi {
namespace tvl1 {

template <int PPL, bool GAM = false>
struct Slot {
    Dyn<PPL> d;
    Stat<PPL> s;
};
template <int PPL>
struct Slot<PPL, true> {
    Dyn<PPL> d;
    Stat<PPL> s;
    Dyn3<PPL> g;
};
template <int PPL> __device__ __forceinline__ Dyn3<PPL> *g3(Slot<PPL, true> &x) { return &x.g; }
template <int PPL> __device__ __forceinline__ Dyn3<PPL> *g3(Slot<PPL, false> &) { return nullptr; }

struct GamK { float gamma, eu3, xl3, xr3; };
template <int PPL, bool ERR, int JW = 0, bool MK = true, bool GAM = false>
__device__ __forceinline__ void stage_r(Dyn<PPL> &A, Dyn<PPL> &B, const Stat<PPL> &st, const bool right_ok[PPL], float negm1,
                                        float m2, float taum2, float l_t, float theta, float taut, unsigned long long &acc, float es,
                                        float xl1 = 0.f, float xl2 = 0.f, float xr1 = 0.f, float xr2 = 0.f, Dyn3<PPL> *A3 = nullptr,
                                        Dyn3<PPL> *B3 = nullptr, const GamK G = GamK{0.f, 0.f, 0.f, 0.f})
{
    float dx1[PPL], dx2[PPL], dx3[PPL];
    dx1[0] = A.p11[0] - (JW ? dpp_from_prev_fill(A.p11[PPL - 1], xl1) : dpp_from_prev(A.p11[PPL - 1]));
    dx2[0] = A.p21[0] - (JW ? dpp_from_prev_fill(A.p21[PPL - 1], xl2) : dpp_from_prev(A.p21[PPL - 1]));
    if constexpr (GAM) dx3[0] = A3->p31[0] - (JW ? dpp_from_prev_fill(A3->p31[PPL - 1], G.xl3) : dpp_from_prev(A3->p31[PPL - 1]));
#pragma unroll
    for (int j = 1; j < PPL; ++j) {
        dx1[j] = A.p11[j] - A.p11[j - 1]; dx2[j] = A.p21[j] - A.p21[j - 1];
        if constexpr (GAM) dx3[j] = A3->p31[j] - A3->p31[j - 1];
    }
    const float r1 = JW ? dpp_from_next_fill(B.u1[0], xr1) : dpp_from_next(B.u1[0]);
    const float r2 = JW ? dpp_from_next_fill(B.u2[0], xr2) : dpp_from_next(B.u2[0]);
    float r3 = 0.f;
    if constexpr (GAM) r3 = JW ? dpp_from_next_fill(B3->u3[0], G.xr3) : dpp_from_next(B3->u3[0]);
#pragma unroll
    for (int j = 0; j < PPL; ++j) {
        const float div1 = dx1[j] + (MK ? fmaf(negm1, B.p12[j], A.p12[j]) : A.p12[j] - B.p12[j]);
        const float div2 = dx2[j] + (MK ? fmaf(negm1, B.p22[j], A.p22[j]) : A.p22[j] - B.p22[j]);
        float rho0 = st.rc[j];
        if constexpr (GAM) rho0 = fmaf(G.gamma, A3->u3[j], rho0);
        const float rho = fmaf(st.ix[j], A.u1[j], fmaf(st.iy[j], A.u2[j], rho0));
        const float fi = __builtin_amdgcn_fmed3f(-rho * st.rg[j], -l_t, l_t);
        const float nu1 = fmaf(theta, div1, fmaf(fi, st.ix[j], A.u1[j]));
        const float nu2 = fmaf(theta, div2, fmaf(fi, st.iy[j], A.u2[j]));
        const float n1 = (j + 1 < PPL) ? B.u1[j + 1 < PPL ? j + 1 : j] : r1;
        const float n2 = (j + 1 < PPL) ? B.u2[j + 1 < PPL ? j + 1 : j] : r2;
        const float u1x = right_ok[j] ? n1 - B.u1[j] : 0.f;
        const float u2x = right_ok[j] ? n2 - B.u2[j] : 0.f;
        const float d1 = nu1 - B.u1[j];
        const float d2 = nu2 - B.u2[j];
        const float g1 = __builtin_amdgcn_sqrtf(MK ? fmaf(d1 * d1, m2, u1x * u1x) : d1 * d1 + u1x * u1x);
        const float g2 = __builtin_amdgcn_sqrtf(MK ? fmaf(d2 * d2, m2, u2x * u2x) : d2 * d2 + u2x * u2x);
        const float q1 = __builtin_amdgcn_rcpf(fmaf(taut, g1, 1.0f));
        const float q2 = __builtin_amdgcn_rcpf(fmaf(taut, g2, 1.0f));
        B.p11[j] = fmaf(taut, u1x, B.p11[j]) * q1;
        B.p12[j] = fmaf(MK ? taum2 : taut, d1, B.p12[j]) * q1;
        B.p21[j] = fmaf(taut, u2x, B.p21[j]) * q2;
        B.p22[j] = fmaf(MK ? taum2 : taut, d2, B.p22[j]) * q2;
        float e3sq = 0.f;
        if constexpr (GAM) {
            const float div3 = dx3[j] + (MK ? fmaf(negm1, B3->p32[j], A3->p32[j]) : A3->p32[j] - B3->p32[j]);
            const float nu3 = fmaf(theta, div3, fmaf(fi, G.gamma, A3->u3[j]));
            const float n3 = (j + 1 < PPL) ? B3->u3[j + 1 < PPL ? j + 1 : j] : r3;
            const float u3x = right_ok[j] ? n3 - B3->u3[j] : 0.f;
            const float d3 = nu3 - B3->u3[j];
            const float g3 = __builtin_amdgcn_sqrtf(MK ? fmaf(d3 * d3, m2, u3x * u3x) : d3 * d3 + u3x * u3x);
            const float q3 = __builtin_amdgcn_rcpf(fmaf(taut, g3, 1.0f));
            B3->p31[j] = fmaf(taut, u3x, B3->p31[j]) * q3;
            B3->p32[j] = fmaf(MK ? taum2 : taut, d3, B3->p32[j]) * q3;
            if (ERR) { const float e3 = nu3 - A3->u3[j]; e3sq = e3 * e3 * G.eu3; }
            A3->u3[j] = nu3;
        }
        if (ERR) {
            const float e1 = nu1 - A.u1[j], e2 = nu2 - A.u2[j];
            const float et = GAM ? fmaf(e1, e1, e2 * e2) + e3sq : fmaf(e1, e1, e2 * e2);
            acc += (unsigned long long)__float2uint_rn(et * es);
        }
        A.u1[j] = nu1;
        A.u2[j] = nu2;
        if (ERR) {
            unsigned lo = (unsigned)acc, hi = (unsigned)(acc >> 32);
            asm volatile("" : "+v"(lo), "+v"(hi), "+v"(A.u1[j]));
            acc = ((unsigned long long)hi << 32) | lo;
        }
    }
}

__device__ __forceinline__ void stage_r_exact(Dyn<1> &A, Dyn<1> &B, const Stat<1> &st, bool right_ok, bool x0, bool top, bool bottom,
                                              float l_t, float theta, float taut)
{
    const float p11l = dpp_from_prev(A.p11[0]), p21l = dpp_from_prev(A.p21[0]);
    const float r1 = dpp_from_next(B.u1[0]), r2 = dpp_from_next(B.u2[0]);
    const float p11 = A.p11[0], p12 = A.p12[0], p21 = A.p21[0], p22 = A.p22[0];
    const float up12 = B.p12[0], up22 = B.p22[0];
    float d1, d2;
    {
        const float a1 = x0 ? p11 : p11 - p11l, a2 = x0 ? p21 : p21 - p21l;
        const float in1 = (p11 - p11l) + (p12 - up12), in2 = (p21 - p21l) + (p22 - up22);
        const float le1 = p11 + p12 - up12, le2 = p21 + p22 - up22;
        const float tp1 = a1 + p12, tp2 = a2 + p22;
        d1 = top ? tp1 : (x0 ? le1 : in1);
        d2 = top ? tp2 : (x0 ? le2 : in2);
    }
    const float ix = st.ix[0], iy = st.iy[0], g = st.rg[0], rc = st.rc[0], u1 = A.u1[0], u2 = A.u2[0];
    const float rho = rc + (ix * u1 + iy * u2);
    const float ltg = l_t * g;
    float e1 = 0.f, e2 = 0.f;
    if (rho < -ltg) { e1 = l_t * ix; e2 = l_t * iy; }
    else if (rho > ltg) { e1 = -l_t * ix; e2 = -l_t * iy; }
    else if (g > 1.1920928955078125e-7f) { const float fi = -rho / g; e1 = fi * ix; e2 = fi * iy; }
    const float v1 = u1 + e1, v2 = u2 + e2;
    const float nu1 = v1 + theta * d1, nu2 = v2 + theta * d2;
    const float u1x = right_ok ? r1 - B.u1[0] : 0.f, u2x = right_ok ? r2 - B.u2[0] : 0.f;
    const float u1y = bottom ? 0.f : nu1 - B.u1[0], u2y = bottom ? 0.f : nu2 - B.u2[0];
    {
        const float gn = (float)sqrt((double)u1x * (double)u1x + (double)u1y * (double)u1y);
        const float ng = 1.0f + taut * gn;
        B.p11[0] = (B.p11[0] + taut * u1x) / ng;
        B.p12[0] = (B.p12[0] + taut * u1y) / ng;
    }
    {
        const float gn = (float)sqrt((double)u2x * (double)u2x + (double)u2y * (double)u2y);
        const float ng = 1.0f + taut * gn;
        B.p21[0] = (B.p21[0] + taut * u2x) / ng;
        B.p22[0] = (B.p22[0] + taut * u2y) / ng;
    }
    A.u1[0] = nu1;
    A.u2[0] = nu2;
}

template <int PPL>
__device__ __forceinline__ void ldr(float dst[PPL], const float *rowp, unsigned xb)
{
    const char *q = reinterpret_cast<const char *>(rowp) + xb;
    if (PPL == 1) {
        dst[0] = *reinterpret_cast<const float *>(q);
    } else if (PPL == 2) {
        const float2 v = *reinterpret_cast<const float2 *>(q);
        dst[0] = v.x; dst[1] = v.y;
    } else {
        const float4 v = *reinterpret_cast<const float4 *>(q);
        dst[0] = v.x; dst[1] = v.y; dst[2] = v.z; dst[3] = v.w;
    }
}
template <int PPL>
__device__ __forceinline__ void str(float *rowp, unsigned xb, const float v[PPL])
{
    char *q = reinterpret_cast<char *>(rowp) + xb;
    if (PPL == 1) *reinterpret_cast<float *>(q) = v[0];
    else if (PPL == 2) *reinterpret_cast<float2 *>(q) = make_float2(v[0], v[1]);
    else *reinterpret_cast<float4 *>(q) = make_float4(v[0], v[1], v[2], v[3]);
}

template <int PPL, bool PZ, bool NG = false, bool P16 = false, int FW = 0, bool GAM = false>
__device__ __forceinline__ void load_row_r(Slot<PPL, GAM> &x, const TbArgs &A, const float *const u[3], const float *const p[6], int row,
                                           int H, unsigned xc)
{
    const long long ro = (long long)min(max(row, 0), H - 1) * A.g.ld;
    asm volatile("" : "+v"(xc));
    if (!FW) {
        ldr<PPL>(x.s.ix, A.pl.ix + ro, xc);
        ldr<PPL>(x.s.iy, A.pl.iy + ro, xc);
        if (!NG) ldr<PPL>(x.s.rg, A.pl.g + ro, xc);
        ldr<PPL>(x.s.rc, A.pl.rc + ro, xc);
    }
    ldr<PPL>(x.d.u1, u[0] + ro, xc);
    ldr<PPL>(x.d.u2, u[1] + ro, xc);
    if (!PZ && P16) {
        ldr<PPL>(x.d.p11, p[0] + ro, xc);
        ldr<PPL>(x.d.p21, p[2] + ro, xc);
    } else if (!PZ) {
        ldr<PPL>(x.d.p11, p[0] + ro, xc);
        ldr<PPL>(x.d.p12, p[1] + ro, xc);
        ldr<PPL>(x.d.p21, p[2] + ro, xc);
        ldr<PPL>(x.d.p22, p[3] + ro, xc);
    } else {
#pragma unroll
        for (int j = 0; j < PPL; ++j) x.d.p11[j] = x.d.p12[j] = x.d.p21[j] = x.d.p22[j] = 0.f;
    }
    if constexpr (GAM) {
        ldr<PPL>(x.g.u3, u[2] + ro, xc);
        if (!PZ) {
            ldr<PPL>(x.g.p31, p[4] + ro, xc);
            ldr<PPL>(x.g.p32, p[5] + ro, xc);
        } else {
#pragma unroll
            for (int j = 0; j < PPL; ++j) x.g.p31[j] = x.g.p32[j] = 0.f;
        }
    }
}

template <int PPL>
struct CtxR {
    TbArgs B;
    const float *uin[3], *pin[6];
    float *uout[3], *pout[6];
    float *ring;
    float *inbox;
    int lane, H, ld, y0, y1, ystart, nsteps;
    unsigned xc;
    bool st_ok, x0;
    bool right_ok[PPL];
    float l_t, theta, taut;
    float gamma, eu3;
    int nit;
};

constexpr int XS = 32;
__host__ __device__ constexpr int xarea_bytes(int T) { return 2 * T * XS; }
__host__ __device__ constexpr int xdump_bytes(int T) { return 2 * T * XS + 64 * 8; }
#define MI_LDS __attribute__((address_space(3)))
typedef MI_LDS char *lds_ptr;
struct Xchg {
    unsigned own, pub_r, pub_l;
    unsigned mul;
    unsigned tag; float l1, l2, r1, r2;
    int budget;
    bool on_r, on_l;
};
__device__ __forceinline__ void xread(unsigned slot, unsigned &tag, float &l1, float &l2, float &r1, float &r2)
{
    const lds_ptr q = (lds_ptr)(unsigned long long)slot;
    tag = *reinterpret_cast<volatile MI_LDS unsigned *>(q + 16);
    const unsigned long long L = *reinterpret_cast<volatile MI_LDS unsigned long long *>(q);
    const unsigned long long R = *reinterpret_cast<volatile MI_LDS unsigned long long *>(q + 8);
    l1 = __uint_as_float((unsigned)L); l2 = __uint_as_float((unsigned)(L >> 32));
    r1 = __uint_as_float((unsigned)R); r2 = __uint_as_float((unsigned)(R >> 32));
}
__device__ __forceinline__ void xwrite(unsigned slot, int data_off, int tag_off, float a, float b, unsigned tag)
{
    const lds_ptr q = (lds_ptr)(unsigned long long)slot;
    *reinterpret_cast<volatile MI_LDS float *>(q + data_off) = a;
    *reinterpret_cast<volatile MI_LDS float *>(q + data_off + 4) = b;
    *reinterpret_cast<volatile MI_LDS unsigned short *>(q + tag_off) = (unsigned short)tag;
}
constexpr int XS2 = 16;
__host__ __device__ constexpr int xs2_bytes(bool gam) { return gam ? 32 : XS2; }
__host__ __device__ constexpr int jw_waves(int JW) { return JW == 3 ? 8 : 4; }
__host__ __device__ constexpr int xk_stages(int T) { return T >= 10 && T % 5 == 0 ? 5 : T >= 4 ? 2 : 1; }
__host__ __device__ constexpr int xarea2_bytes(int T, bool gam = false) { return 2 * T * xs2_bytes(gam); }
__device__ __forceinline__ void xbarrier() { asm volatile("s_waitcnt lgkmcnt(0)\n\ts_barrier" ::: "memory"); }
__device__ __forceinline__ void xread2(unsigned slot, float &l1, float &l2, float &r1, float &r2)
{
    typedef float f4 __attribute__((ext_vector_type(4)));
    const f4 v = *reinterpret_cast<volatile MI_LDS f4 *>((lds_ptr)(unsigned long long)slot);
    l1 = v.x; l2 = v.y; r1 = v.z; r2 = v.w;
}
__device__ __forceinline__ void xwrite2(bool on, unsigned addr, float a, float b)
{
    typedef float f2 __attribute__((ext_vector_type(2)));
    if (on) {
        f2 v; v.x = a; v.y = b;
        *reinterpret_cast<volatile MI_LDS f2 *>((lds_ptr)(unsigned long long)addr) = v;
    }
}
__device__ __forceinline__ void xread1g(unsigned slot, float &l3, float &r3)
{
    typedef float f2 __attribute__((ext_vector_type(2)));
    const f2 v = *reinterpret_cast<volatile MI_LDS f2 *>((lds_ptr)(unsigned long long)(slot + 16));
    l3 = v.x; r3 = v.y;
}
__device__ __forceinline__ void xwrite1(bool on, unsigned addr, float a)
{
    if (on) *reinterpret_cast<volatile MI_LDS float *>((lds_ptr)(unsigned long long)addr) = a;
}
__device__ __forceinline__ void xwrite2f(unsigned addr, float a, float b)
{
    typedef float f2 __attribute__((ext_vector_type(2)));
    f2 v; v.x = a; v.y = b;
    *reinterpret_cast<volatile MI_LDS f2 *>((lds_ptr)(unsigned long long)addr) = v;
}
__host__ __device__ constexpr int xdump4_bytes(int T) { return 64 * 8 + 2 * xarea2_bytes(T) + 64; }
__host__ __device__ constexpr bool jw_fast(int JW) { return JW == 4; }
__device__ int g_jw_fault;

constexpr int FW_RING = 4;
constexpr int FW_SLOT = 3 * 64;
__host__ __device__ constexpr int fw_lds_floats(int NW) { return NW * FW_RING * FW_SLOT + 128; }
template <int PPL>
__device__ __forceinline__ void fw_inbox_get(const float *slot, int lane, Stat<PPL> &s)
{
    const float *q = slot + lane;
    s.ix[0] = q[0]; s.iy[0] = q[64]; s.rc[0] = q[128];
}
template <int FW> struct FwSem { static constexpr int sem = FW == 2 ? MI_SEM_CUDA_COMPAT : MI_SEM_CPU_REF; static constexpr bool fast = FW == 2; };

#ifndef FW_STAGE
#define FW_STAGE 0
#endif
#ifndef FW_X
#define FW_X 0
#endif
struct FwU { float u1, u2, i0; };

template <int FW, int NW>
__device__ __forceinline__ void fw_produce(const TbArgs &A, float *inbox, const float *tab, int lane, int xw, int ystart, int nsteps_total,
                                           long long pb, int cur)
{
    constexpr int SEM = FwSem<FW>::sem;
    constexpr bool FAST = FwSem<FW>::fast;
    const int W = A.g.w, H = A.g.h, ld = A.g.ld;
    const int x = min(xw + lane, W - 1);
    const float *U1 = A.pl.u[cur][0] + pb + x, *U2 = A.pl.u[cur][1] + pb + x, *I0 = A.fI0 + pb + x, *P = A.fI1 + pb;
    FwU U[4];
    float R[2][6][6];
    const auto load_u = [&](int m, FwU &u) {
        const long long ro = (long long)min(max(ystart + m, 0), H - 1) * ld;
#if FW_X == 0
        u.u1 = U1[ro]; u.u2 = U2[ro]; u.i0 = I0[ro];
#else
        u.u1 = u.u2 = 0.25f; u.i0 = (float)ro;
#endif
    };
    const auto gather = [&](int m, const FwU &u, float (&Rw)[6][6]) {
        int sx, sy;
        float wx[4], wy[4];
        warp_coords<SEM>(tab, x, min(max(ystart + m, 0), H - 1), u.u1, u.u2, sx, sy, wx, wy);
#if FW_X == 0
        window_gather(Rw, P, ld, min(max(sx, 1), W - 5), min(max(sy, 1), H - 5));
#else
        for (int r = 0; r < 6; ++r) for (int c = 0; c < 6; ++c) Rw[r][c] = u.u1 + (float)(r * 6 + c);
#endif
    };
    const auto sums = [&](int m, const FwU &u, const float (&Rw)[6][6]) {
        float v0, v1, v2;
#if FW_X == 1
        v0 = v1 = v2 = 0.f;
#else
        int sx, sy;
        float wx[4], wy[4];
        warp_coords<SEM>(tab, x, min(max(ystart + m, 0), H - 1), u.u1, u.u2, sx, sy, wx, wy);
#if FW_X == 2
        window_sums<SEM, FAST>(Rw, wx, wy, v0, v1, v2);
#else
        if (window_interior(sx, sy, W, H)) window_sums<SEM, FAST>(Rw, wx, wy, v0, v1, v2);
        else window_border<SEM>(P, W, H, ld, sx, sy, wx, wy, v0, v1, v2);
#endif
#endif
        float *q = inbox + (m & (FW_RING - 1)) * FW_SLOT + lane;
        q[0] = v1; q[64] = v2;
        q[128] = (v0 - v1 * u.u1 - v2 * u.u2 - u.i0);
    };
#if FW_X == 1
#define FW_ROW(m, k) do { sums((m), U[(k) & 3], R[(k) & 1]); } while (0)
#else
#define FW_ROW(m, k) do { sums((m), U[(k) & 3], R[(k) & 1]); gather((m) + 2, U[((k) + 2) & 3], R[(k) & 1]); load_u((m) + 4, U[(k) & 3]); } while (0)
#endif
    load_u(0, U[0]); load_u(1, U[1]); load_u(2, U[2]); load_u(3, U[3]);
    gather(0, U[0], R[0]); gather(1, U[1], R[1]);
    FW_ROW(0, 0);
    FW_ROW(1, 1);
    xbarrier();
    int n = 0;
#pragma unroll 1
    for (; n + 4 <= nsteps_total; n += 4) {
        xbarrier(); FW_ROW(n + 2, 2); xbarrier();
        xbarrier(); FW_ROW(n + 3, 3); xbarrier();
        xbarrier(); FW_ROW(n + 4, 0); xbarrier();
        xbarrier(); FW_ROW(n + 5, 1); xbarrier();
    }
    if (n < nsteps_total) { xbarrier(); FW_ROW(n + 2, 2); xbarrier(); }
    if (n + 1 < nsteps_total) { xbarrier(); FW_ROW(n + 3, 3); xbarrier(); }
    if (n + 2 < nsteps_total) { xbarrier(); FW_ROW(n + 4, 0); xbarrier(); }
#undef FW_ROW
    for (int i = 0; i < NW - 1; ++i) xbarrier();
}

constexpr int FWS_D1 = 5, FWS_D2 = 8;
constexpr int FWS_CW = 64 + 2 * FWS_D1 + 6;
constexpr int FWS_NR = 2 * FWS_D2 + 6;
__host__ __device__ constexpr int fws_lds_floats(int NW) { return NW * FWS_NR * FWS_CW; }

template <int FW, int NW>
__device__ __forceinline__ void fw_produce_staged(const TbArgs &A, float *inbox, const float *tab, float *ring, int lane, int xw, int ystart,
                                                  int nsteps_total, int y_mid, long long pb, int cur)
{
    constexpr int SEM = FwSem<FW>::sem;
    constexpr bool FAST = FwSem<FW>::fast;
    const int W = A.g.w, H = A.g.h, ld = A.g.ld;
    const int x = min(xw + lane, W - 1);
    const float *U1 = A.pl.u[cur][0] + pb + x, *U2 = A.pl.u[cur][1] + pb + x, *I0 = A.fI0 + pb + x, *P = A.fI1 + pb;
    int ox, oy;
    {
        const long long ro = (long long)min(max(y_mid, 0), H - 1) * ld;
        float a = U1[ro], b = U2[ro];
#pragma unroll
        for (int o = 32; o > 0; o >>= 1) { a += __shfl_xor(a, o); b += __shfl_xor(b, o); }
        ox = __builtin_amdgcn_readfirstlane(__float2int_rn(fminf(fmaxf(a * (1.0f / 64.0f), -30000.f), 30000.f)));
        oy = __builtin_amdgcn_readfirstlane(__float2int_rn(fminf(fmaxf(b * (1.0f / 64.0f), -30000.f), 30000.f)));
    }
    const int cb = xw + ox - FWS_D1 - 3;
    const int ca = min(max(cb + lane, 0), W - 1), cbb = min(max(cb + 64 + lane, 0), W - 1);
    const bool second = lane < FWS_CW - 64;
    FwU U[4];
    float ST[4][2];
    const auto load_u = [&](int m, FwU &u) {
        const long long ro = (long long)min(max(ystart + m, 0), H - 1) * ld;
        u.u1 = U1[ro]; u.u2 = U2[ro]; u.i0 = I0[ro];
    };
    const auto load_row = [&](int r, float (&st)[2]) {
        const float *q = P + (long long)min(max(r, 0), H - 1) * ld;
        st[0] = q[ca];
        st[1] = q[cbb];
    };
    const auto store_row = [&](int slot, const float (&st)[2]) {
        float *q = ring + slot * FWS_CW + lane;
        q[0] = st[0];
        if (second) q[64] = st[1];
    };
    int rlow = ystart + oy - FWS_D2 - 2;
    int slot_low = ((rlow % FWS_NR) + FWS_NR) % FWS_NR;
    for (int r0 = 0; r0 < FWS_NR; r0 += 4) {
#pragma unroll
        for (int k = 0; k < 4; ++k) if (r0 + k < FWS_NR) load_row(rlow + r0 + k, ST[k]);
#pragma unroll
        for (int k = 0; k < 4; ++k) if (r0 + k < FWS_NR) { int sl = slot_low + r0 + k; sl -= sl >= FWS_NR ? FWS_NR : 0; store_row(sl, ST[k]); }
    }
#pragma unroll
    for (int k = 0; k < 4; ++k) load_row(rlow + FWS_NR + k, ST[k]);
    load_u(0, U[0]); load_u(1, U[1]); load_u(2, U[2]); load_u(3, U[3]);

    const auto row = [&](int m, const FwU &u, int rlow_m, int slot_lo) {
        const int yu = ystart + m;
        float v0 = 0.f, v1 = 0.f, v2 = 0.f, rc = 0.f;
        if (yu >= 0 && yu < H) {
            int sx, sy;
            float wx[4], wy[4];
            warp_coords<SEM>(tab, x, yu, u.u1, u.u2, sx, sy, wx, wy);
            const int dc = sx - 1 - cb, dr = sy - 1 - rlow_m;
            const bool inter = window_interior(sx, sy, W, H);
            const bool staged = inter && (unsigned)dc <= (unsigned)(FWS_CW - 6) && (unsigned)dr <= (unsigned)(FWS_NR - 6);
            if (staged) {
                float Rw[6][6];
                unsigned t = (unsigned)(slot_lo + dr);
                t = min(t, t - (unsigned)FWS_NR);
#pragma unroll
                for (int r = 0; r < 6; ++r) {
                    const float *q = ring + t * FWS_CW + dc;
#pragma unroll
                    for (int c = 0; c < 6; ++c)
                        if (!((r == 0 || r == 5) && (c == 0 || c == 5))) Rw[r][c] = q[c];
                    ++t;
                    t = min(t, t - (unsigned)FWS_NR);
                }
                window_sums<SEM, FAST>(Rw, wx, wy, v0, v1, v2);
            } else if (inter) {
                float Rw[6][6];
                window_gather(Rw, P, ld, sx, sy);
                window_sums<SEM, FAST>(Rw, wx, wy, v0, v1, v2);
            } else {
                window_border<SEM>(P, W, H, ld, sx, sy, wx, wy, v0, v1, v2);
            }
            rc = (v0 - v1 * u.u1 - v2 * u.u2 - u.i0);
        }
        float *q = inbox + (m & (FW_RING - 1)) * FW_SLOT + lane;
        q[0] = v1; q[64] = v2; q[128] = rc;
    };
#define FWS_STEP(m, k)                                                                               \
    do {                                                                                             \
        store_row(slot_low, ST[((k) + 3) & 3]);     \
        asm volatile("" ::: "memory");                                                               \
        load_row(rlow + FWS_NR + 4, ST[((k) + 3) & 3]);              \
        ++rlow;                                                                                      \
        slot_low = slot_low + 1 == FWS_NR ? 0 : slot_low + 1;                                        \
        row((m), U[(k) & 3], rlow, slot_low);                                                        \
        load_u((m) + 4, U[(k) & 3]);                                                                 \
    } while (0)
    row(0, U[0], rlow, slot_low);
    load_u(4, U[0]);
    FWS_STEP(1, 1);
    xbarrier();
    int n = 0;
#pragma unroll 1
    for (; n + 4 <= nsteps_total; n += 4) {
        xbarrier(); FWS_STEP(n + 2, 2); xbarrier();
        xbarrier(); FWS_STEP(n + 3, 3); xbarrier();
        xbarrier(); FWS_STEP(n + 4, 0); xbarrier();
        xbarrier(); FWS_STEP(n + 5, 1); xbarrier();
    }
    if (n < nsteps_total) { xbarrier(); FWS_STEP(n + 2, 2); xbarrier(); }
    if (n + 1 < nsteps_total) { xbarrier(); FWS_STEP(n + 3, 3); xbarrier(); }
    if (n + 2 < nsteps_total) { xbarrier(); FWS_STEP(n + 4, 0); xbarrier(); }
#undef FWS_STEP
    for (int i = 0; i < NW - 1; ++i) xbarrier();
}

template <int T, int PPL, bool PZ, int PF, int MODE, int JW, bool MK, bool NG, bool P16, int FW, bool GAM, int k>
__device__ __forceinline__ void step_r(const CtxR<PPL> &c, Slot<PPL, GAM> (&X)[T + 1 + PF], int n0, int &slot0, unsigned long long (&acc)[T], Xchg &x)
{
    constexpr bool JF = jw_fast(JW);
    constexpr int XSg = xs2_bytes(GAM);
    constexpr int XAg = xarea2_bytes(T, GAM);
    constexpr int P = T + 1 + PF;
    constexpr int K = T > 2 ? T - 1 : 1;
    const int n = n0 + k;
    const int r0 = c.ystart + n;
    if (P16 && !PZ) {
#pragma unroll
        for (int j = 0; j < PPL; ++j) {
            const int a = __float_as_int(X[k].d.p11[j]), b = __float_as_int(X[k].d.p21[j]);
            const float sc = 1.0f / 32767.0f;
            X[k].d.p11[j] = (float)(short)(a & 0xffff) * sc; X[k].d.p12[j] = (float)(a >> 16) * sc;
            X[k].d.p21[j] = (float)(short)(b & 0xffff) * sc; X[k].d.p22[j] = (float)(b >> 16) * sc;
        }
    }
    if (NG) {
#pragma unroll
        for (int j = 0; j < PPL; ++j) { const float ix2 = X[k].s.ix[j] * X[k].s.ix[j], iy2 = X[k].s.iy[j] * X[k].s.iy[j]; X[k].s.rg[j] = ix2 + iy2; }
    }
    if (MODE != 2) finish_static<PPL>(X[k].s);
    unsigned xexpect = 0, vtag_r = 0, vtag_l = 0;
    if (JW >= 2) {
        asm volatile("" : "+v"(x.own), "+v"(x.pub_l));
        if (JF) asm volatile("" : "+v"(x.pub_r));
        if (JF) xwrite2f(x.pub_r, X[k].d.p11[0], X[k].d.p21[0]);
        else xwrite2(x.on_r, x.own + XAg, X[k].d.p11[0], X[k].d.p21[0]);
        if constexpr (GAM) xwrite1(x.on_r, x.own + XAg + 16, X[k].g.p31[0]);
    } else if (JW) {
        vtag_r = (unsigned)(n + 1); vtag_l = (unsigned)(n + 2);
        asm volatile("" : "+v"(vtag_r), "+v"(vtag_l), "+v"(x.own));
        xwrite(x.pub_r, 0, 16, X[k].d.p11[0], X[k].d.p21[0], vtag_r);
        xexpect = ((unsigned)(n + 1) & 0xffffu) * x.mul;
    }
#ifndef TBR_X_NOLOAD
    load_row_r<PPL, PZ, NG, P16, FW, GAM>(X[(k + PF) % P], c.B, c.uin, c.pin, r0 + PF, c.H, c.xc);
#else
    X[(k + PF) % P] = X[k];
#endif
    Stat<PPL> nx;
#pragma unroll
    for (int j = 0; j < PPL; ++j) nx.ix[j] = nx.iy[j] = nx.rg[j] = nx.rc[j] = 0.f;
    if (T < 3) lds_put<PPL>(c.ring + slot0 * (256 * PPL), c.lane, X[k].s);
#pragma unroll
    for (int t = 0; t < T; ++t) {
        Stat<PPL> st;
        if (t == 0) st = X[k].s;
        else if (t == 1) st = X[(k - 1 + P) % P].s;
        else st = nx;
#ifdef TBR_X_NOLDS
        if (t >= 2) st = X[k].s;
#else
        if (t + 1 < T && t + 1 >= 2) {
            int sl = slot0 - (t + 1);
            if (sl < 0) sl += K;
            lds_get<PPL>(c.ring + sl * (256 * PPL), c.lane, nx);
            if (t + 1 == T - 1) lds_put<PPL>(c.ring + slot0 * (256 * PPL), c.lane, X[k].s);
        }
#endif
        const int a = r0 - t;
        const float negm1 = MK ? __uint_as_float((a == 0) ? 0u : 0xbf800000u) : -1.f;
        const float m2 = MK ? __uint_as_float((a == c.H) ? 0u : 0x3f800000u) : 1.f;
        const float taum2 = MK ? __uint_as_float((a == c.H) ? 0u : __float_as_uint(c.taut)) : c.taut;
        if (MODE == 1) {
            const float es = __uint_as_float((a >= c.y0 && a < c.y1) ? 0x4b800000u : 0u);
            if (JW >= 2) {
                if ((k * T + t) % xk_stages(T) == 0) xbarrier();
                float l1, l2, r1, r2;
                GamK G{c.gamma, c.eu3, 0.f, 0.f};
                xread2(x.own + t * 2 * XSg, l1, l2, r1, r2);
                if constexpr (GAM) xread1g(x.own + t * 2 * XSg, G.xl3, G.xr3);
                Dyn<PPL> &SA = X[(k - t + P) % P].d, &SB = X[(k - t - 1 + 2 * P) % P].d;
                Dyn3<PPL> *const SA3 = g3(X[(k - t + P) % P]), *const SB3 = g3(X[(k - t - 1 + 2 * P) % P]);
                if (t < c.nit) stage_r<PPL, true, 1, true, GAM>(SA, SB, st, c.right_ok, negm1, m2, taum2, c.l_t, c.theta, c.taut, acc[t], es, l1, l2, r1, r2, SA3, SB3, G);
                if (t + 1 < T) xwrite2(x.on_r, x.own + XAg + (t + 1) * 2 * XSg, SB.p11[0], SB.p21[0]);
                xwrite2(x.on_l, x.pub_l + t * 2 * XSg + 8, SA.u1[0], SA.u2[0]);
                if constexpr (GAM) {
                    if (t + 1 < T) xwrite1(x.on_r, x.own + XAg + (t + 1) * 2 * XSg + 16, SB3->p31[0]);
                    xwrite1(x.on_l, x.pub_l + t * 2 * XSg + 20, SA3->u3[0]);
                }
            } else if (t < c.nit)
                stage_r<PPL, true, 0, true, GAM>(X[(k - t + P) % P].d, X[(k - t - 1 + 2 * P) % P].d, st, c.right_ok, negm1, m2, taum2, c.l_t, c.theta,
                                                 c.taut, acc[t], es, 0.f, 0.f, 0.f, 0.f, g3(X[(k - t + P) % P]), g3(X[(k - t - 1 + 2 * P) % P]),
                                                 GamK{c.gamma, c.eu3, 0.f, 0.f});
        } else if (MODE == 2) {
            if constexpr (PPL == 1)
                stage_r_exact(X[(k - t + P) % P].d, X[(k - t - 1 + 2 * P) % P].d, st, c.right_ok[0], c.x0, a == 0, a == c.H, c.l_t, c.theta, c.taut);
        } else if (JF) {
            constexpr int XKs = xk_stages(T);
            if ((k * T + t) % XKs == 0) xbarrier();
            if (t == 0 || (k * T + t) % XKs == 0) xread2(x.own + t * 2 * XS2, x.l1, x.l2, x.r1, x.r2);
            const float l1 = x.l1, l2 = x.l2, r1 = x.r1, r2 = x.r2;
            if (t + 1 < T && (k * T + t + 1) % XKs != 0) xread2(x.own + (t + 1) * 2 * XS2, x.l1, x.l2, x.r1, x.r2);
            unsigned long long dummy = 0;
            Dyn<PPL> &SA = X[(k - t + P) % P].d, &SB = X[(k - t - 1 + 2 * P) % P].d;
            stage_r<PPL, false, 1, MK>(SA, SB, st, c.right_ok, negm1, m2, taum2, c.l_t, c.theta, c.taut, dummy, 0.f, l1, l2, r1, r2);
            if (t + 1 < T) xwrite2f(x.pub_r + (t + 1) * 2 * XS2, SB.p11[0], SB.p21[0]);
            xwrite2f(x.pub_l + t * 2 * XS2 + 8, SA.u1[0], SA.u2[0]);
        } else if (JW >= 2) {
            if ((k * T + t) % xk_stages(T) == 0) xbarrier();
            if constexpr (FW != 0) if (t == 0) fw_inbox_get<PPL>(c.inbox + ((n + 1) & (FW_RING - 1)) * FW_SLOT, c.lane, X[(k + 1) % P].s);
            float l1, l2, r1, r2;
            GamK G{c.gamma, 0.f, 0.f, 0.f};
            xread2(x.own + t * 2 * XSg, l1, l2, r1, r2);
            if constexpr (GAM) xread1g(x.own + t * 2 * XSg, G.xl3, G.xr3);
            unsigned long long dummy = 0;
            Dyn<PPL> &SA = X[(k - t + P) % P].d, &SB = X[(k - t - 1 + 2 * P) % P].d;
            Dyn3<PPL> *const SA3 = g3(X[(k - t + P) % P]), *const SB3 = g3(X[(k - t - 1 + 2 * P) % P]);
            stage_r<PPL, false, 1, true, GAM>(SA, SB, st, c.right_ok, negm1, m2, taum2, c.l_t, c.theta, c.taut, dummy, 0.f, l1, l2, r1, r2, SA3, SB3, G);
            if (t + 1 < T) xwrite2(x.on_r, x.own + XAg + (t + 1) * 2 * XSg, SB.p11[0], SB.p21[0]);
            xwrite2(x.on_l, x.pub_l + t * 2 * XSg + 8, SA.u1[0], SA.u2[0]);
            if constexpr (GAM) {
                if (t + 1 < T) xwrite1(x.on_r, x.own + XAg + (t + 1) * 2 * XSg + 16, SB3->p31[0]);
                xwrite1(x.on_l, x.pub_l + t * 2 * XSg + 20, SA3->u3[0]);
            }
        } else if (JW) {
            unsigned tag = x.tag;
            float l1 = x.l1, l2 = x.l2, r1 = x.r1, r2 = x.r2;
#pragma nounroll
            while (__builtin_amdgcn_readfirstlane(tag) != xexpect) {
                __builtin_amdgcn_s_sleep(1);
                xread(x.own + t * XS, tag, l1, l2, r1, r2);
                if (--x.budget < 0) xexpect = __builtin_amdgcn_readfirstlane(tag);
            }
            if (t + 1 < T) xread(x.own + (t + 1) * XS, x.tag, x.l1, x.l2, x.r1, x.r2);
            else xread(x.own + ((n & 1) ? -T * XS : T * XS), x.tag, x.l1, x.l2, x.r1, x.r2);
            unsigned long long dummy = 0;
            Dyn<PPL> &SA = X[(k - t + P) % P].d, &SB = X[(k - t - 1 + 2 * P) % P].d;
            stage_r<PPL, false, 1>(SA, SB, st, c.right_ok, negm1, m2, taum2, c.l_t, c.theta, c.taut, dummy, 0.f, l1, l2, r1, r2);
            if (t + 1 < T) xwrite(x.pub_r + (t + 1) * XS, 0, 16, SB.p11[0], SB.p21[0], vtag_r);
            xwrite(x.pub_l + t * XS, 8, 18, SA.u1[0], SA.u2[0], vtag_l);
        } else {
            unsigned long long dummy = 0;
            stage_r<PPL, false, 0, true, GAM>(X[(k - t + P) % P].d, X[(k - t - 1 + 2 * P) % P].d, st, c.right_ok, negm1, m2, taum2, c.l_t, c.theta,
                                              c.taut, dummy, 0.f, 0.f, 0.f, 0.f, 0.f, g3(X[(k - t + P) % P]), g3(X[(k - t - 1 + 2 * P) % P]),
                                              GamK{c.gamma, 0.f, 0.f, 0.f});
        }
    }
    if (JW >= 2) {
        x.own ^= XSg; x.pub_l ^= XSg;
        if (JF) x.pub_r ^= XSg;
    } else if (JW) {
        const int d = (n & 1) ? -T * XS : T * XS;
        x.own += d; x.pub_r += d; x.pub_l -= d;
    }
    {
        const Dyn<PPL> &r = X[(k - T + 2 * P) % P].d;
        const int orow = r0 - T;
#ifdef TBR_X_NOSTORE
        if (orow == c.y1 - 1 && c.st_ok) {
#else
        if (orow >= c.y0 && orow < c.y1 && c.st_ok) {
#endif
            const long long ro = (long long)orow * c.ld;
            unsigned xb = c.xc;
            asm volatile("" : "+v"(xb));
            str<PPL>(c.uout[0] + ro, xb, r.u1);
            str<PPL>(c.uout[1] + ro, xb, r.u2);
            if (P16 && !c.B.skip_p_out) {
                float pa[PPL], pb2[PPL];
#pragma unroll
                for (int j = 0; j < PPL; ++j) {
                    typedef short s2 __attribute__((ext_vector_type(2)));
                    const s2 v1 = __builtin_amdgcn_cvt_pknorm_i16(r.p11[j], r.p12[j]), v2 = __builtin_amdgcn_cvt_pknorm_i16(r.p21[j], r.p22[j]);
                    pa[j] = __int_as_float(((int)(unsigned short)v1.x) | ((int)v1.y << 16));
                    pb2[j] = __int_as_float(((int)(unsigned short)v2.x) | ((int)v2.y << 16));
                }
                str<PPL>(c.pout[0] + ro, xb, pa);
                str<PPL>(c.pout[2] + ro, xb, pb2);
            } else if (!c.B.skip_p_out) {
                str<PPL>(c.pout[0] + ro, xb, r.p11);
                str<PPL>(c.pout[1] + ro, xb, r.p12);
                str<PPL>(c.pout[2] + ro, xb, r.p21);
                str<PPL>(c.pout[3] + ro, xb, r.p22);
            }
            if constexpr (GAM) {
                const Dyn3<PPL> &r3 = X[(k - T + 2 * P) % P].g;
                str<PPL>(c.uout[2] + ro, xb, r3.u3);
                if (!c.B.skip_p_out) {
                    str<PPL>(c.pout[4] + ro, xb, r3.p31);
                    str<PPL>(c.pout[5] + ro, xb, r3.p32);
                }
            }
        }
    }
    slot0 = (slot0 + 1 == K) ? 0 : slot0 + 1;
}
template <int T, int PPL, bool PZ, int PF, int MODE, int JW, bool MK, bool NG, bool P16, int FW, bool GAM, int... Ks>
__device__ __forceinline__ void steps_r(const CtxR<PPL> &c, Slot<PPL, GAM> (&X)[T + 1 + PF], int n0, int &slot0, unsigned long long (&acc)[T],
                                        Xchg &x, std::integer_sequence<int, Ks...>)
{
    (step_r<T, PPL, PZ, PF, MODE, JW, MK, NG, P16, FW, GAM, Ks>(c, X, n0, slot0, acc, x), ...);
}

template <int T, int PPL, bool PZ, int WPS, int PF, int MODE, int JW = 0, bool NG = false, bool P16 = false, int FW = 0, bool GAM = false>
__global__ __launch_bounds__((JW == 3 || FW) ? 512 : 256, WPS) void k_iterate_tbr(TbArgs A)
{
    static_assert(!GAM || (NG && !P16 && !FW && (JW == 0 || JW == 2) && MODE != 2), "illumination channel: independent or barrier-joined waves, fast math, no |grad|^2 plane");
    static_assert(!FW || (JW == 2 && MODE == 0 && NG && !P16 && PPL == 1 && T == 10), "fused warp: the default joined-wave fixed-work kernel only");
    static_assert(!JW || (PPL == 1 && T > 2 && (MODE == 0 || (MODE == 1 && JW >= 2 && JW != 4))), "joined waves: 1 px per lane; the speculative steps in the barrier form only");
    static_assert(JW < 2 || (((T + 1 + PF) * T) % xk_stages(T) == 0 && T >= 2 * xk_stages(T)), "barrier intervals must tile the unrolled block and leave the right neighbour a full interval");
    constexpr int M = (T + PPL - 1) / PPL * PPL;
    constexpr int NW = jw_waves(JW);
    constexpr int LW = (JW ? 64 * NW : 64) * PPL;
    constexpr int STRIDE = LW - 2 * M;
    constexpr int P = T + 1 + PF;
    constexpr int K = T > 2 ? T - 1 : 1;
    extern __shared__ __attribute__((aligned(16))) float lds[];
    CtxR<PPL> c;
    c.lane = threadIdx.x & 63;
    const int wave_id = __builtin_amdgcn_readfirstlane(threadIdx.x >> 6);
    const bool producer = FW && wave_id >= NW;
    const int wave = producer ? wave_id - NW : wave_id;
    int strip = blockIdx.x, bgrp = blockIdx.y, b = blockIdx.z;
    if (A.swz & 1) {
        const unsigned nwg = gridDim.x * gridDim.y * gridDim.z;
        const unsigned orig = blockIdx.x + gridDim.x * (blockIdx.y + gridDim.y * blockIdx.z);
        const unsigned xcd = orig & 7u, qq = nwg >> 3, rr = nwg & 7u;
        const unsigned lid = (xcd < rr ? xcd * (qq + 1) : rr * (qq + 1) + (xcd - rr) * qq) + (orig >> 3);
        strip = lid % gridDim.x; bgrp = (lid / gridDim.x) % gridDim.y; b = lid / (gridDim.x * gridDim.y);
    }
    strip = __builtin_amdgcn_readfirstlane(strip); bgrp = __builtin_amdgcn_readfirstlane(bgrp); b = __builtin_amdgcn_readfirstlane(b);
    const int band = JW ? bgrp : bgrp * 4 + wave;
    const int W = A.g.w;
    c.H = A.g.h; c.ld = A.g.ld;
    c.y0 = band * A.rows_per_band;
    c.ring = lds + wave * (K * 256 * PPL);
    if (c.y0 >= c.H) return;
    c.y1 = min(c.y0 + A.rows_per_band, c.H);
    const int own_lo = strip == 0 ? 0 : (LW - M) + (strip - 1) * STRIDE;
    const int own_hi = min(strip == 0 ? LW - M : own_lo + STRIDE, W);
    const int xw = (strip == 0 ? 0 : own_lo - M) + (JW ? wave * 64 : 0);
    const int xl = xw + c.lane * PPL;
    Xchg x;
    x.own = x.pub_r = x.pub_l = 0; x.mul = 0; x.tag = 0; x.l1 = x.l2 = x.r1 = x.r2 = 0.f; x.budget = 1 << 20; x.on_r = x.on_l = false;
    if (JW >= 2) {
        constexpr int XA = xarea2_bytes(T, GAM);
        const unsigned xb = (unsigned)(unsigned long long)(lds_ptr)(lds + NW * (K * 256 * PPL));
        const bool has_left = wave > 0, has_right = wave < NW - 1 && xw + 64 < W;
        x.own = xb + wave * XA;
        x.pub_l = xb + (wave - 1) * XA + xs2_bytes(GAM);
        x.on_r = has_right && c.lane == 63;
        x.on_l = has_left && c.lane == 0;
        if (FW && threadIdx.x < 128) (lds + NW * (K * 256 * PPL) + NW * XA / 4 + NW * FW_RING * FW_SLOT)[threadIdx.x] = A.ftab[threadIdx.x];
        if (jw_fast(JW)) {
            const unsigned dump = xb + NW * XA + 32 + c.lane * 8;
            x.pub_r = x.on_r ? x.own + XA : dump;
            x.pub_l = x.on_l ? x.pub_l : dump;
        }
        for (int i = c.lane; i < XA / 4; i += 64) reinterpret_cast<volatile MI_LDS unsigned *>((lds_ptr)(unsigned long long)x.own)[i] = 0u;
        __syncthreads();
        if (xw >= W) return;
    } else if (JW) {
        constexpr int XA = xarea_bytes(T), XD = xdump_bytes(T);
        const unsigned xb = (unsigned)(unsigned long long)(lds_ptr)(lds + 4 * (K * 256 * PPL));
        const bool has_left = wave > 0, has_right = wave < 3 && xw + 64 < W;
        const unsigned dump = xb + 4 * XA + wave * XD + c.lane * 8;
        x.own = xb + wave * XA;
        x.pub_r = (has_right && c.lane == 63) ? xb + (wave + 1) * XA : dump;
        x.pub_l = ((has_left && c.lane == 0) ? xb + (wave - 1) * XA : dump) + T * XS;
        x.mul = (has_left ? 1u : 0u) | (has_right ? 0x10000u : 0u);
        for (int i = c.lane; i < XA / 4; i += 64) {
            const int w4 = i % (XS / 4), buf = i / (T * XS / 4);
            reinterpret_cast<volatile MI_LDS unsigned *>((lds_ptr)(unsigned long long)x.own)[i] = (w4 == 4 && buf == 0 && has_right) ? 0x10000u : 0u;
        }
        __syncthreads();
        if (xw >= W) return;
    }
#pragma unroll
    for (int j = 0; j < PPL; ++j) c.right_ok[j] = (xl + j + 1 < W);
    c.st_ok = xl >= own_lo && xl < own_hi;
    c.x0 = xl == 0;
    c.xc = 4u * (unsigned)min(xl, c.ld - PPL);

    const long long pb = (long long)b * A.g.ps;
    int cur = A.cur;
    c.ystart = c.y0 - T;
    c.nsteps = (c.y1 - c.y0) + 2 * T;
    c.inbox = nullptr;
    if constexpr (FW != 0) {
        float *fw0 = lds + NW * (K * 256 * PPL) + NW * xarea2_bytes(T) / 4;
        c.inbox = fw0 + wave * (FW_RING * FW_SLOT);
        if (producer) {
#if FW_STAGE
            fw_produce_staged<FW, NW>(A, c.inbox, fw0 + NW * FW_RING * FW_SLOT, fw0 + fw_lds_floats(NW) + wave * (FWS_NR * FWS_CW), c.lane, xw, c.ystart,
                                      (c.nsteps + P - 1) / P * P, (c.y0 + c.y1) >> 1, pb, cur);
#else
            fw_produce<FW, NW>(A, c.inbox, fw0 + NW * FW_RING * FW_SLOT, c.lane, xw, c.ystart, (c.nsteps + P - 1) / P * P, pb, cur);
#endif
            return;
        }
    }
    c.nit = T;
    bool record = false;
    if (MODE == 1) {
        int nit = 0;
        if (!spec_settle(A.ctl, A.sk, T, b, strip == 0 && bgrp == 0 && threadIdx.x == 0, cur, nit, record)) return;
        c.nit = __builtin_amdgcn_readfirstlane(nit);
    }
    c.uin[0] = A.pl.u[cur][0] + pb; c.uin[1] = A.pl.u[cur][1] + pb;
    c.uout[0] = A.pl.u[cur ^ 1][0] + pb; c.uout[1] = A.pl.u[cur ^ 1][1] + pb;
#pragma unroll
    for (int i = 0; i < 4; ++i) { c.pin[i] = A.pl.p[cur][i] + pb; c.pout[i] = A.pl.p[cur ^ 1][i] + pb; }
    c.uin[2] = nullptr; c.uout[2] = nullptr; c.pin[4] = c.pin[5] = nullptr; c.pout[4] = c.pout[5] = nullptr;
    c.gamma = 0.f; c.eu3 = 0.f;
    if constexpr (GAM) {
        c.uin[2] = A.pl.u[cur][2] + pb; c.uout[2] = A.pl.u[cur ^ 1][2] + pb;
#pragma unroll
        for (int i = 4; i < 6; ++i) { c.pin[i] = A.pl.p[cur][i] + pb; c.pout[i] = A.pl.p[cur ^ 1][i] + pb; }
        c.gamma = A.pl.gamma; c.eu3 = A.pl.err_u3 ? 1.f : 0.f;
    }
    c.B = A;
    if (!FW) { c.B.pl.ix += pb; c.B.pl.iy += pb; if (!NG) c.B.pl.g += pb; c.B.pl.rc += pb; }
    c.l_t = A.l_t; c.theta = A.theta; c.taut = A.taut;

    Slot<PPL, GAM> X[P];
#pragma unroll
    for (int i = 0; i < P; ++i)
#pragma unroll
        for (int j = 0; j < PPL; ++j) {
            X[i].d.u1[j] = X[i].d.u2[j] = X[i].d.p11[j] = X[i].d.p12[j] = X[i].d.p21[j] = X[i].d.p22[j] = 0.f;
            X[i].s.ix[j] = X[i].s.iy[j] = X[i].s.rg[j] = X[i].s.rc[j] = 0.f;
            if constexpr (GAM) X[i].g.u3[j] = X[i].g.p31[j] = X[i].g.p32[j] = 0.f;
        }
    for (int k = 0; k < K; ++k) lds_put<PPL>(c.ring + k * (256 * PPL), c.lane, X[0].s);

#pragma unroll
    for (int k = 0; k < PF; ++k) load_row_r<PPL, PZ, NG, P16, FW, GAM>(X[k], c.B, c.uin, c.pin, c.ystart + k, c.H, c.xc);
    if constexpr (FW != 0) {
        xbarrier();
        fw_inbox_get<PPL>(c.inbox, c.lane, X[0].s);
    }
    int slot0 = 0;
    unsigned long long acc[T];
#pragma unroll
    for (int t = 0; t < T; ++t) acc[t] = 0;
    if (JW >= 2 && xk_stages(T) > 1)
        for (int i = 0; i < wave; ++i) xbarrier();
    for (int n0 = 0; n0 < c.nsteps; n0 += P) {
        if (jw_fast(JW)) {
            const int ra = c.ystart + n0 - (T - 1), rb = c.ystart + n0 + P - 1;
            const bool plain = (ra > 0 || rb < 0) && (ra > c.H || rb < c.H);
            if (plain) { steps_r<T, PPL, PZ, PF, MODE, JW, false, NG, P16, FW, GAM>(c, X, n0, slot0, acc, x, std::make_integer_sequence<int, P>{}); continue; }
        }
        steps_r<T, PPL, PZ, PF, MODE, JW, true, NG, P16, FW, GAM>(c, X, n0, slot0, acc, x, std::make_integer_sequence<int, P>{});
    }
    if (JW >= 2 && xk_stages(T) > 1)
        for (int i = wave; i < NW - 1; ++i) xbarrier();
    if (JW == 1 && x.budget < 0 && c.lane == 0) g_jw_fault = 1;
    if (MODE == 1 && record) {
#pragma unroll
        for (int t = 0; t < T; ++t) {
            unsigned long long sacc = c.st_ok ? acc[t] : 0ull;
#pragma unroll
            for (int o = 32; o > 0; o >>= 1) sacc += __shfl_xor(sacc, o);
            if (c.lane == 0 && t < c.nit) atomicAdd(&A.ctl.E[(long long)b * A.ctl.Q + A.e0 + t], sacc);
        }
    }
}

template <int T, int PPL, int WPS, int PF, int MODE, int JW = 0, bool NG = false, bool P16 = false, int FW = 0, bool GAM = false>
static int launch_tbr(const TbArgs &A0, bool pz, hipStream_t s)
{
    constexpr int M = (T + PPL - 1) / PPL * PPL;
    constexpr int NW = jw_waves(JW);
    constexpr int LW = (JW ? 64 * NW : 64) * PPL;
    constexpr int STRIDE = LW - 2 * M;
    TbArgs A = A0;
    A.nstrips = A.g.w <= LW - M ? 1 : 1 + div_up(A.g.w - (LW - M), STRIDE);
    A.swz = tuning().tb_swz == 1 ? 1 : 0;
    const dim3 grid(A.nstrips, JW ? div_up(A.g.h, A.rows_per_band) : div_up(div_up(A.g.h, A.rows_per_band), 4), A.g.batch);
    constexpr size_t lds_bytes = (size_t)NW * (T > 2 ? T - 1 : 1) * 256 * PPL * sizeof(float) +
                                 (JW >= 2 ? NW * xarea2_bytes(T, GAM) + (jw_fast(JW) ? xdump4_bytes(T) : 0) : JW ? 4 * (xarea_bytes(T) + xdump_bytes(T)) : 0) +
                                 (FW ? (fw_lds_floats(NW) + (FW_STAGE ? fws_lds_floats(NW) : 0)) * sizeof(float) : 0);
    constexpr int NTHREADS = 64 * NW * (FW ? 2 : 1);
    static const hipError_t attr_rc = [] {
        hipError_t e = hipFuncSetAttribute((const void *)k_iterate_tbr<T, PPL, true, WPS, PF, MODE, JW, NG, P16, FW, GAM>, hipFuncAttributeMaxDynamicSharedMemorySize, (int)lds_bytes);
        if (e == hipSuccess)
            e = hipFuncSetAttribute((const void *)k_iterate_tbr<T, PPL, false, WPS, PF, MODE, JW, NG, P16, FW, GAM>, hipFuncAttributeMaxDynamicSharedMemorySize, (int)lds_bytes);
        return e;
    }();
    MI_HIP_TRY(attr_rc);
    if (tuning().tb_verbose) {
        static const int nb = [] {
            int n = -1;
            (void)hipOccupancyMaxActiveBlocksPerMultiprocessor(&n, (const void *)k_iterate_tbr<T, PPL, false, WPS, PF, MODE, JW, NG, P16, FW, GAM>, NTHREADS, lds_bytes);
            fprintf(stderr, "[tbr] T=%d ppl=%d wps=%d pf=%d jw=%d lds=%zu B/block -> %d resident blocks/CU\n", T, PPL, WPS, PF, JW, lds_bytes, n);
            return n;
        }();
        (void)nb;
    }
    if (pz) hipLaunchKernelGGL((k_iterate_tbr<T, PPL, true, WPS, PF, MODE, JW, NG, P16, FW, GAM>), grid, dim3(NTHREADS), lds_bytes, s, A);
    else hipLaunchKernelGGL((k_iterate_tbr<T, PPL, false, WPS, PF, MODE, JW, NG, P16, FW, GAM>), grid, dim3(NTHREADS), lds_bytes, s, A);
    MI_HIP_TRY(hipGetLastError());
    return MI_OK;
}

typedef int (*TbLaunchFn)(const TbArgs &, bool, hipStream_t);
struct TbrEntry {
    int T, PPL, WPS, PF, PLAN;
    TbLaunchFn launch, spec;
    int JW;
    bool GAM;
};
#define TBR(T, PPL, WPS, PF, PLAN) {T, PPL, WPS, PF, PLAN, launch_tbr<T, PPL, WPS, PF, 0>, nullptr, 0}
static const TbrEntry g_tbr_jw[] = {
#ifdef MIFLOW_EXPERIMENTS
                                     {10, 1, 3, 2, 3, launch_tbr<10, 1, 3, 2, 0, 1>, nullptr, 1},
                                     {10, 1, 4, 2, 3, launch_tbr<10, 1, 4, 2, 0, 3>, nullptr, 3},
                                     {10, 1, 4, 2, 3, launch_tbr<10, 1, 4, 2, 0, 4>, nullptr, 4},
#endif
                                     {10, 1, 4, 2, 3, launch_tbr<10, 1, 4, 2, 0, 2>, nullptr, 2}};
static const TbrEntry g_tbr_ng = {10, 1, 4, 2, 3, launch_tbr<10, 1, 4, 2, 0, 2, true>, nullptr, 2};
#ifdef MIFLOW_EXPERIMENTS
static const TbrEntry g_tbr_fw[] = {{10, 1, 4, 2, 2, launch_tbr<10, 1, 4, 2, 0, 2, true, false, 1>, nullptr, 2},
                                    {10, 1, 4, 2, 2, launch_tbr<10, 1, 4, 2, 0, 2, true, false, 2>, nullptr, 2}};
#endif
static const TbrEntry g_tbr_gam[] = {{10, 1, 3, 1, 3, launch_tbr<10, 1, 3, 1, 0, 2, true, false, 0, true>, nullptr, 2, true},
                                     {5, 1, 4, 2, 3, launch_tbr<5, 1, 4, 2, 0, 2, true, false, 0, true>, nullptr, 2, true},
                                     {2, 1, 6, 2, 6, launch_tbr<2, 1, 6, 2, 0, 0, true, false, 0, true>, nullptr, 0, true},
                                     {1, 1, 8, 2, 8, launch_tbr<1, 1, 8, 2, 0, 0, true, false, 0, true>, nullptr, 0, true}};
static const TbrEntry g_spec_gam[] = {{10, 1, 2, 2, 2, nullptr, launch_tbr<10, 1, 2, 2, 1, 2, true, false, 0, true>, 2, true},
                                      {5, 1, 3, 2, 2, nullptr, launch_tbr<5, 1, 3, 2, 1, 2, true, false, 0, true>, 2, true}};
#ifdef MIFLOW_EXPERIMENTS
static const TbrEntry g_tbr_ng16 = {10, 1, 4, 2, 3, launch_tbr<10, 1, 4, 2, 0, 2, true, true>, nullptr, 2};
#endif
static const TbrEntry g_tbr[] = {
    TBR(10, 1, 4, 2, 3), TBR(8, 2, 2, 2, 2), TBR(6, 1, 5, 2, 3), TBR(5, 2, 3, 2, 3), TBR(4, 2, 3, 2, 3), TBR(3, 1, 7, 2, 6), TBR(2, 1, 8, 2, 8),
    TBR(1, 1, 8, 2, 8),
#ifdef MIFLOW_EXPERIMENTS
    TBR(10, 2, 2, 2, 2), TBR(8, 1, 4, 2, 2), TBR(6, 2, 3, 2, 3),
#endif
};
#define TBRS(T, PPL, WPS, PF, PLAN) {T, PPL, WPS, PF, PLAN, nullptr, launch_tbr<T, PPL, WPS, PF, 1>, 0}
#define TBRSJ(T, PPL, WPS, PF, PLAN) {T, PPL, WPS, PF, PLAN, nullptr, launch_tbr<T, PPL, WPS, PF, 1, 2>, 2}
#ifdef MIFLOW_EXPERIMENTS
static const TbrEntry g_spec[] = {TBRS(10, 1, 3, 2, 2), TBRS(5, 1, 4, 2, 2)};
static const TbrEntry g_spec_jw[] = {TBRSJ(10, 1, 3, 2, 2), TBRSJ(5, 1, 4, 2, 2)};
#endif
static const TbrEntry g_spec_jw_ng[] = {{10, 1, 3, 2, 2, nullptr, launch_tbr<10, 1, 3, 2, 1, 2, true>, 2}, {5, 1, 4, 2, 2, nullptr, launch_tbr<5, 1, 4, 2, 1, 2, true>, 2}};

#define TBRX(T, WPS, PLAN) {T, 1, WPS, 2, PLAN, launch_tbr<T, 1, WPS, 2, 2>, nullptr, 0}
static const TbrEntry g_exact[] = {TBRX(5, 4, 3), TBRX(4, 4, 3), TBRX(3, 5, 4), TBRX(2, 6, 4), TBRX(1, 8, 4)};

static const TbrEntry *tbr_pick(int T)
{
    const Tuning &tn = tuning();
    if (tn.tb_jw && tn.tb_ppl < 0)
        for (const TbrEntry &e : g_tbr_jw)
            if (e.T == T && e.JW == tn.tb_jw) return &e;
    const TbrEntry *def = nullptr;
    for (const TbrEntry &e : g_tbr) {
        if (e.T != T) continue;
        if (!def) def = &e;
        if (e.PPL == tn.tb_ppl && e.WPS == tn.tb_wps && e.PF == tn.tb_pf) { def = &e; break; }
    }
    return def;
}

static int plan_band_rows(const TbrEntry &e, const Geo &g)
{
    const Tuning &tn = tuning();
    if (tn.tb_rows > 0) return tn.tb_rows;
    const int T = e.T, ppl = e.PPL, P = T + 1 + e.PF;
    int wps = e.PLAN;
    const int ring_slots = T > 2 ? T - 1 : 1;
    const int nw = e.JW ? jw_waves(e.JW) : 4;
    int lds_blocks = (160 * 1024) / (ring_slots * nw * 256 * ppl * 4 + (e.JW >= 2 ? nw * xarea2_bytes(T, e.GAM) + (jw_fast(e.JW) ? xdump4_bytes(T) : 0) : e.JW ? 4 * (xarea_bytes(T) + xdump_bytes(T)) : 0));
    lds_blocks = lds_blocks * nw / 4;
    if (wps > lds_blocks) wps = lds_blocks;
    if (tn.tb_plan_wps > 0) wps = tn.tb_plan_wps;
    const long long cap = (long long)device_simds() * wps;
    const int M = (T + ppl - 1) / ppl * ppl;
    const int LW = (e.JW ? 64 * nw : 64) * ppl;
    const long long strips = g.w <= LW - M ? 1 : 1 + div_up(g.w - (LW - M), LW - 2 * M);
    const long long per_band = strips * g.batch * (e.JW ? nw : 1);
    long long best_cost = -1;
    int best_nb = 1;
    for (int nb = 1; nb <= g.h; ++nb) {
        const int R = div_up(g.h, nb);
        if (R < 8 && nb > 1) break;
        const long long cap_nb = !e.JW && nb < 4 && nb < wps ? (long long)device_simds() * nb : cap;
        const long long rounds = (per_band * nb + cap_nb - 1) / cap_nb;
        const long long steps = (long long)div_up(R + 2 * T, P) * P;
        const long long cost = rounds * steps;
        if (best_cost < 0 || cost < best_cost) { best_cost = cost; best_nb = nb; }
    }
    return div_up(g.h, best_nb);
}

int tb_query_plan(int T, const Geo &g, int *kernel, int *rows)
{
    if (runs_on_tiles(g, T, tv_knobs())) {
        *kernel = 1;
        *rows = tile_owned_rows();
        return MI_OK;
    }
    const TbrEntry *e = tbr_pick(T);
    if (!e) { set_error("unsupported time block %d", T); return MI_ERR_BAD_ARG; }
    *kernel = 0;
    *rows = plan_band_rows(*e, g);
    return MI_OK;
}

int iterate_tb_fused(int semantics, const float *I0, const float *I1, const float *cubic_tab_dev, int T, const IterPlanes &pl, const Geo &g,
                     float l_t, float theta, float taut, bool p_zero, int cur, hipStream_t s, bool skip_p_out)
{
#ifndef MIFLOW_EXPERIMENTS
    (void)semantics; (void)I0; (void)I1; (void)cubic_tab_dev; (void)T; (void)pl; (void)g; (void)l_t; (void)theta; (void)taut; (void)p_zero; (void)cur; (void)s; (void)skip_p_out;
    set_error("the warp fused into the pass kernel exists in the experiments build only (-DMIFLOW_EXPERIMENTS)");
    return MI_ERR_NOT_IMPL;
#else
    MI_REQUIRE(T == 10 && tb_nograd_ok(T, g, tv_knobs()), MI_ERR_BAD_ARG, "fused warp: one pass of the default T = 10 kernel only");
    const TbrEntry &e = g_tbr_fw[semantics == MI_SEM_CPU_REF ? 0 : 1];
    TbArgs A;
    memset(&A, 0, sizeof(A));
    A.pl = pl; A.pl.ix = A.pl.iy = A.pl.g = A.pl.rc = nullptr;
    A.g = g; A.l_t = l_t; A.theta = theta; A.taut = taut; A.cur = cur;
    A.skip_p_out = skip_p_out ? 1 : 0;
    A.fI0 = I0; A.fI1 = I1; A.ftab = cubic_tab_dev;
    A.rows_per_band = plan_band_rows(e, g);
    if (tuning().tb_verbose) {
        static int shown = 0;
        if (shown++ < 40) fprintf(stderr, "[tb] fused warp T=%d %dx%d batch=%d rows_per_band=%d\n", T, g.w, g.h, g.batch, A.rows_per_band);
    }
    return e.launch(A, p_zero, s);
#endif
}

int iterate_tb(int T, const IterPlanes &pl, const Geo &g, float l_t, float theta, float taut, bool p_zero,
               int cur, int rows_per_band, hipStream_t s, bool skip_p_out, bool independent_waves)
{
    if (pl.gamma != 0.f && rows_per_band == 0 && runs_on_tiles(g, T, tv_knobs()))
        return iterate_tile(-1, T, pl, g, l_t, theta, taut, p_zero, cur, s);
    if (pl.gamma != 0.f) {
        const TbrEntry *e = nullptr;
        for (const TbrEntry &c : g_tbr_gam) if (c.T == T) e = &c;
        if (!e) { set_error("gamma != 0: unsupported time block %d", T); return MI_ERR_BAD_ARG; }
        MI_REQUIRE(pl.u[0][2] && pl.u[1][2] && pl.p[0][4] && pl.p[0][5] && pl.p[1][4] && pl.p[1][5], MI_ERR_BAD_ARG, "gamma != 0 needs the u3 / p31 / p32 planes");
        TbArgs A;
        memset(&A, 0, sizeof(A));
        A.pl = pl; A.g = g; A.l_t = l_t; A.theta = theta; A.taut = taut; A.cur = cur;
        A.skip_p_out = skip_p_out ? 1 : 0;
        A.rows_per_band = rows_per_band > 0 ? rows_per_band : plan_band_rows(*e, g);
        return e->launch(A, p_zero, s);
    }
    if (rows_per_band == 0 && runs_on_tiles(g, T, tv_knobs())) {
        MI_REQUIRE(pl.g, MI_ERR_BAD_ARG, "the register-tile kernel needs the |grad|^2 plane");
        return iterate_tile(-1, T, pl, g, l_t, theta, taut, p_zero, cur, s);
    }
    const TbrEntry *e = tbr_pick(T);
    if (independent_waves) {
        e = nullptr;
        for (const TbrEntry &c : g_tbr) if (c.T == T && !e) e = &c;
    }
    if (!e) { set_error("unsupported time block %d", T); return MI_ERR_BAD_ARG; }
    if (!pl.g) {
        MI_REQUIRE(!independent_waves && (rows_per_band != 0 ? T == 10 : tb_nograd_ok(T, g, tv_knobs())), MI_ERR_BAD_ARG,
                   "no |grad|^2 plane, but the kernel of this launch needs one");
#ifdef MIFLOW_EXPERIMENTS
        e = tuning().tb_p16 ? &g_tbr_ng16 : &g_tbr_ng;
#else
        e = &g_tbr_ng;
#endif
    }
    TbArgs A;
    A.pl = pl; A.g = g; A.l_t = l_t; A.theta = theta; A.taut = taut; A.cur = cur; A.swz = 0; A.nstrips = 0;
    A.skip_p_out = skip_p_out ? 1 : 0;
    A.rows_per_band = rows_per_band > 0 ? rows_per_band : plan_band_rows(*e, g);
    if (tuning().tb_verbose) {
        static int shown = 0;
        if (shown++ < 40)
            fprintf(stderr, "[tb] T=%d ppl=%d wps=%d pf=%d %dx%d batch=%d rows_per_band=%d\n", T, e->PPL, e->WPS, e->PF, g.w, g.h, g.batch,
                    A.rows_per_band);
    }
    return e->launch(A, p_zero, s);
}

int iterate_tb_exact(int T, const IterPlanes &pl, const Geo &g, float l_t, float theta, float taut, bool p_zero, int cur, hipStream_t s,
                     int rows_per_band)
{
    const TbrEntry *e = nullptr;
    for (const TbrEntry &c : g_exact) if (c.T == T) e = &c;
    if (!e) { set_error("no exact-math kernel for time block %d", T); return MI_ERR_BAD_ARG; }
    TbArgs A;
    memset(&A, 0, sizeof(A));
    A.pl = pl; A.g = g; A.l_t = l_t; A.theta = theta; A.taut = taut; A.cur = cur;
    A.rows_per_band = rows_per_band > 0 ? rows_per_band : plan_band_rows(*e, g);
    return e->launch(A, p_zero, s);
}

bool tb_kernel_exists(int kind, int T, bool gam, bool nograd)
{
    auto in = [T](const TbrEntry *t, size_t n, bool spec) {
        for (size_t i = 0; i < n; ++i) if (t[i].T == T && (spec ? t[i].spec : t[i].launch)) return true;
        return false;
    };
#define TB_IN(tab, spec) in(tab, sizeof(tab) / sizeof(tab[0]), spec)
    switch (kind) {
    case 0: return gam ? TB_IN(g_tbr_gam, false) : nograd ? T == g_tbr_ng.T : tbr_pick(T) != nullptr;
    case 1: {
        if (nograd) return false;
        if (!gam) return TB_IN(g_tbr, false);
        for (const TbrEntry &c : g_tbr_gam) if (c.T == T && c.JW == 0) return true;
        return false;
    }
    case 2: return !gam && !nograd && TB_IN(g_exact, false);
    case 3: return gam ? TB_IN(g_spec_gam, true) : TB_IN(g_spec_jw_ng, true);
    }
#undef TB_IN
    return false;
}

int iterate_tb_spec(int T, const IterPlanes &pl, const Geo &g, float l_t, float theta, float taut, bool p_zero, const Ctl &ctl,
                    const SpecK &sk, int e0, hipStream_t s, int rows_per_band)
{
    if (rows_per_band == 0 && runs_on_tiles(g, T, tv_knobs(), true) && !p_zero)
        return iterate_tile_spec(T, pl, g, l_t, theta, taut, ctl, sk, e0, s);
    const TbrEntry *e = nullptr;
    if (pl.gamma != 0.f) {
        for (const TbrEntry &c : g_spec_gam) if (c.T == T) e = &c;
    } else if (!pl.g) {
        MI_REQUIRE(rows_per_band != 0 || tb_spec_nograd_ok(g, tv_knobs()), MI_ERR_BAD_ARG,
                   "no |grad|^2 plane, but the speculative kernel of this launch needs one");
        for (const TbrEntry &c : g_spec_jw_ng) if (c.T == T) e = &c;
    }
#ifdef MIFLOW_EXPERIMENTS
    else if (tuning().tb_jw >= 2 && tuning().tb_jw_spec) { for (const TbrEntry &c : g_spec_jw) if (c.T == T) e = &c; }
    else { for (const TbrEntry &c : g_spec) if (c.T == T) e = &c; }
#else
    else for (const TbrEntry &c : g_spec_jw_ng) if (c.T == T) e = &c;
#endif
    if (!e) { set_error("no speculative kernel for time block %d", T); return MI_ERR_BAD_ARG; }
    TbArgs A;
    A.pl = pl; A.g = g; A.l_t = l_t; A.theta = theta; A.taut = taut; A.cur = 0; A.swz = 0; A.nstrips = 0; A.skip_p_out = 0;
    A.rows_per_band = rows_per_band > 0 ? rows_per_band : plan_band_rows(*e, g);
    A.ctl = make_ctlk(&ctl);
    A.e0 = e0;
    A.sk = sk;
    return e->spec(A, p_zero, s);
}

int tb_jw_fault(int *fault_host)
{
    int cur = 0, n = 0, any = 0;
    MI_HIP_TRY(hipGetDevice(&cur));
    MI_HIP_TRY(hipGetDeviceCount(&n));
    for (int d = 0; d < n; ++d) {
        int f = 0;
        if (hipSetDevice(d) != hipSuccess) continue;
        const hipError_t e = hipMemcpyFromSymbol(&f, HIP_SYMBOL(g_jw_fault), sizeof(int), 0, hipMemcpyDeviceToHost);
        if (e != hipSuccess) { (void)hipSetDevice(cur); MI_HIP_TRY(e); }
        any |= f;
    }
    MI_HIP_TRY(hipSetDevice(cur));
    *fault_host = any;
    return MI_OK;
}

__global__ void k_dbg_lane_shift(int *out)
{
    const int l = threadIdx.x;
    out[l] = __float_as_int(dpp_from_prev(__int_as_float(l + 100)));
    out[64 + l] = __float_as_int(dpp_from_next(__int_as_float(l + 100)));
}
int dbg_lane_shift(int *out_dev, hipStream_t s)
{
    hipLaunchKernelGGL(k_dbg_lane_shift, dim3(1), dim3(64), 0, s, out_dev);
    MI_HIP_TRY(hipGetLastError());
    return MI_OK;
}

}
}
```

Measured before the change: 1394 pairs/s.

## Fuse final flow packing into last TV-L1 pass, trim fill steps, rebalance bands

When the plan allows it, the last streaming time-blocked pass at the finest scale writes u1/u2 straight into the interleaved output flow matrix. This removes the separate pack_flow kernel and its extra read and write of the flow planes. The first pipeline block also uses a fill-phase variant that skips time steps on rows still warming up, which removes redundant LDS reads and compute. Band row planning now picks an unequal row split to cut the total wave steps. These add more template instantiations and byte-offset stores with a 32-bit pitch limit.

```diff
diff --git a/opencv_contrib_amd/csrc/mi_common.cpp b/opencv_contrib_amd/csrc/mi_common.cpp
--- a/opencv_contrib_amd/csrc/mi_common.cpp
+++ b/opencv_contrib_amd/csrc/mi_common.cpp
@@ -70,6 +70,8 @@
         t.tb_force = EXP_ENV("MIFLOW_TB_FORCE") != nullptr;
         t.tb_plan_wps = EXP_INT("MIFLOW_TB_WPS", 0);
         t.tb_rows = EXP_INT("MIFLOW_TB_ROWS", 0);
+        t.tb_rows_equal = EXP_INT("MIFLOW_TB_ROWS_EQUAL", 0);
+        t.tb_il = EXP_INT("MIFLOW_TB_IL", 1);
         t.tb_verbose = getenv("MIFLOW_TB_VERBOSE") != nullptr;
         {
             const char *e = getenv("MIFLOW_TILE_MAXPX");
diff --git a/opencv_contrib_amd/csrc/mi_common.h b/opencv_contrib_amd/csrc/mi_common.h
--- a/opencv_contrib_amd/csrc/mi_common.h
+++ b/opencv_contrib_amd/csrc/mi_common.h
@@ -47,6 +47,8 @@
     int tb_force;
     int tb_plan_wps;
     int tb_rows;
+    int tb_rows_equal;
+    int tb_il;
     int tb_verbose;
     long long tile_maxpx;
     int tile_spec;
diff --git a/opencv_contrib_amd/csrc/tvl1_api.cpp b/opencv_contrib_amd/csrc/tvl1_api.cpp
--- a/opencv_contrib_amd/csrc/tvl1_api.cpp
+++ b/opencv_contrib_amd/csrc/tvl1_api.cpp
@@ -303,6 +303,7 @@
         v.tile_fb_block = t.tile_fb_block; v.tile_fb_model = t.tile_fb_model;
         v.tb_force = t.tb_force != 0; v.tb_nograd = t.tb_nograd; v.tb_jw = t.tb_jw; v.tb_ppl = t.tb_ppl; v.tb_jw_spec = t.tb_jw_spec;
         v.tb_fw = t.tb_fw; v.tb_skip_p = t.tb_skip_p; v.tb_hist = t.tb_hist; v.spec = t.spec; v.exact_tb = t.exact_tb;
+        v.tb_il_mask = t.tb_il ? tb_interleave_mask() : 0u;
         v.fb_poll = t.fb_poll; v.fb_ahead = t.fb_ahead; v.warp_fast = t.warp_fast; v.warp_lds = t.warp_lds; v.x_skip = t.x_skip;
         return v;
     }();
@@ -445,7 +446,8 @@
             rc = w.form == TvForm::ExactBlocked ? iterate_tb_exact(w.blocks[k], r.planes, Lv.g, r.l_t, r.theta, r.taut, r.first_of_scale, r.cur, r.st)
                : w.fused ? iterate_tb_fused(sem, Lv.I0, Lv.I1, r.h->cubic_tab, w.blocks[k], r.planes, Lv.g, r.l_t, r.theta, r.taut,
                                             r.first_of_scale, r.cur, r.st, last_pass)
-                         : iterate_tb(w.blocks[k], r.planes, Lv.g, r.l_t, r.theta, r.taut, r.first_of_scale, r.cur, 0, r.st, last_pass);
+                         : iterate_tb(w.blocks[k], r.planes, Lv.g, r.l_t, r.theta, r.taut, r.first_of_scale, r.cur, 0, r.st, last_pass, false,
+                                      last_pass && w.pack_in_pass ? r.ln.tab.p : nullptr);
             if (rc) return rc;
             r.cur ^= 1;
             r.first_of_scale = false;
@@ -648,6 +650,7 @@
     ec.q_prev = r.q_last;
     const Ctl *dev = r.pl.check && !r.first_of_scale ? &ec : nullptr;
     if (s == 0) {
+        if (!r.pl.warp[0].empty() && r.pl.warp[0].back().pack_in_pass) return MI_OK;
         const float *u1v[2] = {Lv.u[0][0], Lv.u[1][0]}, *u2v[2] = {Lv.u[0][1], Lv.u[1][1]};
         return pack_flow(r.ln.tab.p, u1v, u2v, Lv.g, dev, r.cur, r.st);
     }
@@ -681,6 +684,8 @@
     const TvPlan pl = tv_make_plan(TvShape{I0s[0].cols, I0s[0].rows, n, I0s[0].type, P, h->last_lanes, capturing}, tv_knobs());
     int rc = ensure_arena(P, ln, pl, I0s[0].cols, I0s[0].rows, n);
     if (rc || (rc = ensure_buffers(pl, ln, n, I0s, I1s, flows, st))) return rc;
+    if (!pl.warp.empty() && !pl.warp[0].empty() && pl.warp[0].back().pack_in_pass)
+        for (int i = 0; i < n; ++i) MI_REQUIRE(flows[i].step < (1ll << 31), MI_ERR_BAD_ARG, "flow matrix pitch of %lld bytes", (long long)flows[i].step);
     *ns_out = pl.used;
     ln.slots.clear();
     ln.regions.clear();
diff --git a/opencv_contrib_amd/csrc/tvl1_dev.h b/opencv_contrib_amd/csrc/tvl1_dev.h
--- a/opencv_contrib_amd/csrc/tvl1_dev.h
+++ b/opencv_contrib_amd/csrc/tvl1_dev.h
@@ -63,7 +63,8 @@
             bool p_zero, const Ctl *ctl, int cur_host, hipStream_t s);
 
 int iterate_tb(int T, const IterPlanes &pl, const Geo &g, float l_t, float theta, float taut, bool p_zero,
-               int cur, int rows_per_band, hipStream_t s, bool skip_p_out = false, bool independent_waves = false);
+               int cur, int rows_per_band, hipStream_t s, bool skip_p_out = false, bool independent_waves = false,
+               const PtrTab *out_tab = nullptr);
 int iterate_tb_fused(int semantics, const float *I0, const float *I1, const float *cubic_tab_dev, int T, const IterPlanes &pl, const Geo &g,
                      float l_t, float theta, float taut, bool p_zero, int cur, hipStream_t s, bool skip_p_out);
 int iterate_tile(int variant, int nit, const IterPlanes &pl, const Geo &g, float l_t, float theta, float taut, bool p_zero, int cur,
@@ -72,6 +73,7 @@
 int tile_shape_rows(int variant);
 int tb_query_plan(int T, const Geo &g, int *kernel, int *rows);
 int tile_variants();
+unsigned tb_interleave_mask();
 int iterate_tb_exact(int T, const IterPlanes &pl, const Geo &g, float l_t, float theta, float taut, bool p_zero, int cur, hipStream_t s,
                      int rows_per_band = 0);
 bool tb_kernel_exists(int kind, int T, bool gam, bool nograd);
diff --git a/opencv_contrib_amd/csrc/tvl1_plan.h b/opencv_contrib_amd/csrc/tvl1_plan.h
--- a/opencv_contrib_amd/csrc/tvl1_plan.h
+++ b/opencv_contrib_amd/csrc/tvl1_plan.h
@@ -30,6 +30,7 @@
     int tb_nograd, tb_jw, tb_ppl, tb_jw_spec;
     int tb_fw;
     int tb_skip_p, tb_hist, spec, exact_tb;
+    unsigned tb_il_mask;
     int fb_poll, fb_ahead;
     int warp_fast, warp_lds, x_skip;
 };
@@ -111,6 +112,54 @@
     return blocks;
 }
 
+struct TbBandShape {
+    int T, PF, H;
+    long long per_band;
+    long long cap;
+    long long simds;
+    int wps;
+};
+inline long long tb_band_wave_steps(int T, int PF, int rows)
+{
+    const int P = T + 1 + PF;
+    return (long long)((rows + 2 * T + P - 1) / P) * P;
+}
+inline long long tb_band_sum_steps(int T, int PF, int H, int R)
+{
+    const int nb = (H + R - 1) / R;
+    return (nb - 1) * tb_band_wave_steps(T, PF, R) + tb_band_wave_steps(T, PF, H - (nb - 1) * R);
+}
+inline int tb_band_count(const TbBandShape &b)
+{
+    long long best_cost = -1;
+    int best_nb = 1;
+    for (int nb = 1; nb <= b.H; ++nb) {
+        const int R = (b.H + nb - 1) / nb;
+        if (R < 8 && nb > 1) break;
+        const long long cap_nb = b.simds > 0 && nb < 4 && nb < b.wps ? b.simds * nb : b.cap;
+        const long long rounds = (b.per_band * nb + cap_nb - 1) / cap_nb;
+        const long long cost = rounds * tb_band_wave_steps(b.T, b.PF, R);
+        if (best_cost < 0 || cost < best_cost) { best_cost = cost; best_nb = nb; }
+    }
+    return best_nb;
+}
+inline int tb_band_rows_equal(const TbBandShape &b) { const int nb = tb_band_count(b); return (b.H + nb - 1) / nb; }
+inline int tb_band_rows(const TbBandShape &b)
+{
+    const int nb = tb_band_count(b);
+    const int R0 = (b.H + nb - 1) / nb;
+    if (nb == 1) return R0;
+    const long long tallest = tb_band_wave_steps(b.T, b.PF, R0);
+    int best = R0;
+    long long best_sum = tb_band_sum_steps(b.T, b.PF, b.H, R0);
+    for (int R = R0 + 1; (long long)(nb - 1) * R < b.H; ++R) {
+        if (tb_band_wave_steps(b.T, b.PF, R) > tallest) break;
+        const long long sum = tb_band_sum_steps(b.T, b.PF, b.H, R);
+        if (sum < best_sum) { best_sum = sum; best = R; }
+    }
+    return best;
+}
+
 
 struct TvShape {
     int W, H, B, type;
@@ -136,6 +185,7 @@
     bool warp_launch;
     bool skip_iterations;
     bool skip_p_last;
+    bool pack_in_pass;
 };
 
 constexpr size_t kNoPlane = (size_t)-1;
@@ -302,6 +352,11 @@
                 x.blocks = spec_list[x.on_tiles ? 3 : wp > 0 ? 2 : ((double)g.w * g.h * B >= kLargeLevel ? 0 : 1)];
             x.warp_launch = !x.fused && !(K.x_skip == 1 && wp > 0);
             x.skip_p_last = x.form == TvForm::Blocked && K.tb_skip_p && wp == P.warps - 1 && !p.median;
+            if (s == 0 && x.skip_p_last && !gam && !x.fused && !x.skip_iterations && !P.use_initial_flow && !x.blocks.empty()) {
+                const int tl = x.blocks.back();
+                x.pack_in_pass = !runs_on_tiles(g, tl, K) && tl < 31 &&
+                                 ((x.nograd ? K.tb_il_mask >> 31 : K.tb_il_mask >> tl) & 1u) != 0;
+            }
         }
     }
     return p;
diff --git a/opencv_contrib_amd/csrc/tvl1_tb_dev.h b/opencv_contrib_amd/csrc/tvl1_tb_dev.h
--- a/opencv_contrib_amd/csrc/tvl1_tb_dev.h
+++ b/opencv_contrib_amd/csrc/tvl1_tb_dev.h
@@ -44,6 +44,7 @@
     int cur;
     int swz, nstrips;
     int skip_p_out;
+    const PtrTab *otab;
     CtlK ctl;
     int e0;
     SpecK sk;
diff --git a/opencv_contrib_amd/csrc/tvl1_tbr_kernels.hip b/opencv_contrib_amd/csrc/tvl1_tbr_kernels.hip
--- a/opencv_contrib_amd/csrc/tvl1_tbr_kernels.hip
+++ b/opencv_contrib_amd/csrc/tvl1_tbr_kernels.hip
@@ -1,5 +1,6 @@
 #include "tvl1_tb_dev.h"
 #include "tvl1_warp_px.h"
+#include <type_traits>
 #include <utility>
 #include <cstdlib>
 #include <cstdio>
@@ -207,6 +208,8 @@
     float *ring;
     float *inbox;
     int lane, H, ld, y0, y1, ystart, nsteps;
+    int ostep;
+    int osh;
     unsigned xc;
     bool st_ok, x0;
     bool right_ok[PPL];
@@ -494,7 +497,14 @@
     for (int i = 0; i < NW - 1; ++i) xbarrier();
 }
 
-template <int T, int PPL, bool PZ, int PF, int MODE, int JW, bool MK, bool NG, bool P16, int FW, bool GAM, int k>
+__host__ __device__ constexpr bool tb_il_form(int PPL, int JW, bool NG) { return PPL == 1 && (NG || JW == 0); }
+
+__host__ __device__ constexpr bool tb_fill_form(int T, int PPL, bool PZ, int MODE, int JW, bool NG, bool GAM)
+{
+    return MODE != 1 && JW != 1 && !(T == 10 && JW == 2 && !NG && !PZ && !GAM) && !(T == 5 && PPL == 2 && !PZ);
+}
+
+template <int T, int PPL, bool PZ, int PF, int MODE, int JW, bool MK, bool NG, bool P16, int FW, bool GAM, bool FILLB, int k>
 __device__ __forceinline__ void step_r(const CtxR<PPL> &c, Slot<PPL, GAM> (&X)[T + 1 + PF], int n0, int &slot0, unsigned long long (&acc)[T], Xchg &x)
 {
     constexpr bool JF = jw_fast(JW);
@@ -502,6 +512,8 @@
     constexpr int XAg = xarea2_bytes(T, GAM);
     constexpr int P = T + 1 + PF;
     constexpr int K = T > 2 ? T - 1 : 1;
+    constexpr bool FILL = FILLB && tb_fill_form(T, PPL, PZ, MODE, JW, NG, GAM);
+    constexpr int TL = !FILL ? T : (k + 1) / 2 < T ? (k + 1) / 2 : T;
     const int n = n0 + k;
     const int r0 = c.ystart + n;
     if (P16 && !PZ) {
@@ -541,7 +553,7 @@
     for (int j = 0; j < PPL; ++j) nx.ix[j] = nx.iy[j] = nx.rg[j] = nx.rc[j] = 0.f;
     if (T < 3) lds_put<PPL>(c.ring + slot0 * (256 * PPL), c.lane, X[k].s);
 #pragma unroll
-    for (int t = 0; t < T; ++t) {
+    for (int t = 0; t < TL; ++t) {
         Stat<PPL> st;
         if (t == 0) st = X[k].s;
         else if (t == 1) st = X[(k - 1 + P) % P].s;
@@ -550,9 +562,11 @@
         if (t >= 2) st = X[k].s;
 #else
         if (t + 1 < T && t + 1 >= 2) {
-            int sl = slot0 - (t + 1);
-            if (sl < 0) sl += K;
-            lds_get<PPL>(c.ring + sl * (256 * PPL), c.lane, nx);
+            if (t + 1 < TL) {
+                int sl = slot0 - (t + 1);
+                if (sl < 0) sl += K;
+                lds_get<PPL>(c.ring + sl * (256 * PPL), c.lane, nx);
+            }
             if (t + 1 == T - 1) lds_put<PPL>(c.ring + slot0 * (256 * PPL), c.lane, X[k].s);
         }
 #endif
@@ -635,6 +649,14 @@
                                               GamK{c.gamma, 0.f, 0.f, 0.f});
         }
     }
+#pragma unroll
+    for (int t = TL; t < T; ++t) {
+        if (JW >= 2 && (k * T + t) % xk_stages(T) == 0) xbarrier();
+        if constexpr (FW != 0) if (t == 0) fw_inbox_get<PPL>(c.inbox + ((n + 1) & (FW_RING - 1)) * FW_SLOT, c.lane, X[(k + 1) % P].s);
+#ifndef TBR_X_NOLDS
+        if (t + 1 == T - 1 && t + 1 >= 2) lds_put<PPL>(c.ring + slot0 * (256 * PPL), c.lane, X[k].s);
+#endif
+    }
     if (JW >= 2) {
         x.own ^= XSg; x.pub_l ^= XSg;
         if (JF) x.pub_r ^= XSg;
@@ -652,9 +674,20 @@
 #endif
             const long long ro = (long long)orow * c.ld;
             unsigned xb = c.xc;
-            asm volatile("" : "+v"(xb));
-            str<PPL>(c.uout[0] + ro, xb, r.u1);
-            str<PPL>(c.uout[1] + ro, xb, r.u2);
+            if constexpr (!(MODE == 0 && tb_il_form(PPL, JW, NG))) asm volatile("" : "+v"(xb));
+            if constexpr (MODE == 0 && tb_il_form(PPL, JW, NG)) {
+                const long long rou = (long long)orow * c.ostep;
+                unsigned xu = c.xc << c.osh;
+                asm volatile("" : "+v"(xu));
+                typedef __attribute__((address_space(1))) char *gchar_ptr;
+                typedef __attribute__((address_space(1))) float *gfloat_ptr;
+                *reinterpret_cast<gfloat_ptr>((gchar_ptr)reinterpret_cast<char *>(c.uout[0]) + rou + xu) = r.u1[0];
+                *reinterpret_cast<gfloat_ptr>((gchar_ptr)reinterpret_cast<char *>(c.uout[1]) + rou + xu) = r.u2[0];
+                asm volatile("" : "+v"(xb));
+            } else {
+                str<PPL>(c.uout[0] + ro, xb, r.u1);
+                str<PPL>(c.uout[1] + ro, xb, r.u2);
+            }
             if (P16 && !c.B.skip_p_out) {
                 float pa[PPL], pb2[PPL];
 #pragma unroll
@@ -684,11 +717,11 @@
     }
     slot0 = (slot0 + 1 == K) ? 0 : slot0 + 1;
 }
-template <int T, int PPL, bool PZ, int PF, int MODE, int JW, bool MK, bool NG, bool P16, int FW, bool GAM, int... Ks>
+template <int T, int PPL, bool PZ, int PF, int MODE, int JW, bool MK, bool NG, bool P16, int FW, bool GAM, bool FILLB, int... Ks>
 __device__ __forceinline__ void steps_r(const CtxR<PPL> &c, Slot<PPL, GAM> (&X)[T + 1 + PF], int n0, int &slot0, unsigned long long (&acc)[T],
                                         Xchg &x, std::integer_sequence<int, Ks...>)
 {
-    (step_r<T, PPL, PZ, PF, MODE, JW, MK, NG, P16, FW, GAM, Ks>(c, X, n0, slot0, acc, x), ...);
+    (step_r<T, PPL, PZ, PF, MODE, JW, MK, NG, P16, FW, GAM, FILLB, Ks>(c, X, n0, slot0, acc, x), ...);
 }
 
 template <int T, int PPL, bool PZ, int WPS, int PF, int MODE, int JW = 0, bool NG = false, bool P16 = false, int FW = 0, bool GAM = false>
@@ -800,6 +833,12 @@
     c.uout[0] = A.pl.u[cur ^ 1][0] + pb; c.uout[1] = A.pl.u[cur ^ 1][1] + pb;
 #pragma unroll
     for (int i = 0; i < 4; ++i) { c.pin[i] = A.pl.p[cur][i] + pb; c.pout[i] = A.pl.p[cur ^ 1][i] + pb; }
+    c.ostep = 4 * c.ld; c.osh = 0;
+    if (MODE == 0 && tb_il_form(PPL, JW, NG) && A.otab) {
+        c.uout[0] = reinterpret_cast<float *>(A.otab[b].out);
+        c.uout[1] = c.uout[0] + 1;
+        c.ostep = (int)A.otab[b].step_out; c.osh = 1;
+    }
     c.uin[2] = nullptr; c.uout[2] = nullptr; c.pin[4] = c.pin[5] = nullptr; c.pout[4] = c.pout[5] = nullptr;
     c.gamma = 0.f; c.eu3 = 0.f;
     if constexpr (GAM) {
@@ -835,14 +874,18 @@
     for (int t = 0; t < T; ++t) acc[t] = 0;
     if (JW >= 2 && xk_stages(T) > 1)
         for (int i = 0; i < wave; ++i) xbarrier();
-    for (int n0 = 0; n0 < c.nsteps; n0 += P) {
+    const auto block = [&](auto fill, int n0) {
+        constexpr bool FILLB = decltype(fill)::value;
         if (jw_fast(JW)) {
             const int ra = c.ystart + n0 - (T - 1), rb = c.ystart + n0 + P - 1;
             const bool plain = (ra > 0 || rb < 0) && (ra > c.H || rb < c.H);
-            if (plain) { steps_r<T, PPL, PZ, PF, MODE, JW, false, NG, P16, FW, GAM>(c, X, n0, slot0, acc, x, std::make_integer_sequence<int, P>{}); continue; }
-        }
-        steps_r<T, PPL, PZ, PF, MODE, JW, true, NG, P16, FW, GAM>(c, X, n0, slot0, acc, x, std::make_integer_sequence<int, P>{});
-    }
+            if (plain) { steps_r<T, PPL, PZ, PF, MODE, JW, false, NG, P16, FW, GAM, FILLB>(c, X, n0, slot0, acc, x, std::make_integer_sequence<int, P>{}); return; }
+        }
+        steps_r<T, PPL, PZ, PF, MODE, JW, true, NG, P16, FW, GAM, FILLB>(c, X, n0, slot0, acc, x, std::make_integer_sequence<int, P>{});
+    };
+    int n0 = 0;
+    if constexpr (tb_fill_form(T, PPL, PZ, MODE, JW, NG, GAM)) { block(std::true_type{}, 0); n0 = P; }
+    for (; n0 < c.nsteps; n0 += P) block(std::false_type{}, n0);
     if (JW >= 2 && xk_stages(T) > 1)
         for (int i = wave; i < NW - 1; ++i) xbarrier();
     if (JW == 1 && x.budget < 0 && c.lane == 0) g_jw_fault = 1;
@@ -960,7 +1003,7 @@
 {
     const Tuning &tn = tuning();
     if (tn.tb_rows > 0) return tn.tb_rows;
-    const int T = e.T, ppl = e.PPL, P = T + 1 + e.PF;
+    const int T = e.T, ppl = e.PPL;
     int wps = e.PLAN;
     const int ring_slots = T > 2 ? T - 1 : 1;
     const int nw = e.JW ? jw_waves(e.JW) : 4;
@@ -973,18 +1016,22 @@
     const int LW = (e.JW ? 64 * nw : 64) * ppl;
     const long long strips = g.w <= LW - M ? 1 : 1 + div_up(g.w - (LW - M), LW - 2 * M);
     const long long per_band = strips * g.batch * (e.JW ? nw : 1);
-    long long best_cost = -1;
-    int best_nb = 1;
-    for (int nb = 1; nb <= g.h; ++nb) {
-        const int R = div_up(g.h, nb);
-        if (R < 8 && nb > 1) break;
-        const long long cap_nb = !e.JW && nb < 4 && nb < wps ? (long long)device_simds() * nb : cap;
-        const long long rounds = (per_band * nb + cap_nb - 1) / cap_nb;
-        const long long steps = (long long)div_up(R + 2 * T, P) * P;
-        const long long cost = rounds * steps;
-        if (best_cost < 0 || cost < best_cost) { best_cost = cost; best_nb = nb; }
-    }
-    return div_up(g.h, best_nb);
+    const TbBandShape b{T, e.PF, g.h, per_band, cap, e.JW ? 0ll : (long long)device_simds(), wps};
+#ifdef MIFLOW_EXPERIMENTS
+    if (tn.tb_rows_equal) return tb_band_rows_equal(b);
+#endif
+    return tb_band_rows(b);
+}
+
+unsigned tb_interleave_mask()
+{
+    unsigned m = 0;
+    for (int T = 1; T <= kTbMaxBlock; ++T) {
+        const TbrEntry *e = tbr_pick(T);
+        if (e && tb_il_form(e->PPL, e->JW, false)) m |= 1u << T;
+    }
+    if (tb_il_form(g_tbr_ng.PPL, g_tbr_ng.JW, true)) m |= 1u << 31;
+    return m;
 }
 
 int tb_query_plan(int T, const Geo &g, int *kernel, int *rows)
@@ -1027,8 +1074,10 @@
 }
 
 int iterate_tb(int T, const IterPlanes &pl, const Geo &g, float l_t, float theta, float taut, bool p_zero,
-               int cur, int rows_per_band, hipStream_t s, bool skip_p_out, bool independent_waves)
-{
+               int cur, int rows_per_band, hipStream_t s, bool skip_p_out, bool independent_waves, const PtrTab *out_tab)
+{
+    MI_REQUIRE(!out_tab || (skip_p_out && pl.gamma == 0.f && (rows_per_band != 0 || !runs_on_tiles(g, T, tv_knobs()))), MI_ERR_BAD_ARG,
+               "the interleaved store exists in the last streaming pass of a scale without the illumination channel only");
     if (pl.gamma != 0.f && rows_per_band == 0 && runs_on_tiles(g, T, tv_knobs()))
         return iterate_tile(-1, T, pl, g, l_t, theta, taut, p_zero, cur, s);
     if (pl.gamma != 0.f) {
@@ -1062,9 +1111,11 @@
         e = &g_tbr_ng;
 #endif
     }
+    MI_REQUIRE(!out_tab || tb_il_form(e->PPL, e->JW, !pl.g), MI_ERR_BAD_ARG, "the kernel of this launch has no interleaved store");
     TbArgs A;
     A.pl = pl; A.g = g; A.l_t = l_t; A.theta = theta; A.taut = taut; A.cur = cur; A.swz = 0; A.nstrips = 0;
     A.skip_p_out = skip_p_out ? 1 : 0;
+    A.otab = out_tab;
     A.rows_per_band = rows_per_band > 0 ? rows_per_band : plan_band_rows(*e, g);
     if (tuning().tb_verbose) {
         static int shown = 0;
@@ -1131,7 +1182,7 @@
 #endif
     if (!e) { set_error("no speculative kernel for time block %d", T); return MI_ERR_BAD_ARG; }
     TbArgs A;
-    A.pl = pl; A.g = g; A.l_t = l_t; A.theta = theta; A.taut = taut; A.cur = 0; A.swz = 0; A.nstrips = 0; A.skip_p_out = 0;
+    A.pl = pl; A.g = g; A.l_t = l_t; A.theta = theta; A.taut = taut; A.cur = 0; A.swz = 0; A.nstrips = 0; A.skip_p_out = 0; A.otab = nullptr;
     A.rows_per_band = rows_per_band > 0 ? rows_per_band : plan_band_rows(*e, g);
     A.ctl = make_ctlk(&ctl);
     A.e0 = e0;
```

Result: faster. 1454 pairs/s, median of 6 (+4.3%).
